# northflank-examples/distributed-pytorch-example

Hardware: AMD Instinct MI355X
Metric: samples/sec (whole node) + DDP scaling eff., ResNet-50 bf16 at 1/2/4/8 MI355X (higher is better)
Workload: dtype bf16; 1 GPU; model=resnet50-v1.5, global_batch=512, per_gpu_batch=512, grad_accum=1, parallelism=dp1, optimizer=sgd-momentum0.9

## Files before the change

### csrc/bindings/bn.cpp

```cpp
#include <algorithm>
#include <vector>

#include "../kernels/pwconv.h"
#include "gemm_plan.h"
#include "ops_common.h"

namespace dpe_ops {
namespace {

int64_t rows_of(const Tensor& x) { return x.numel() / x.size(-1); }

std::vector<Tensor> bn_fwd_train(const Tensor& x, const c10::optional<Tensor>& gamma, const c10::optional<Tensor>& beta,
                                 const c10::optional<Tensor>& rmean, const c10::optional<Tensor>& rvar, double momentum,
                                 double eps, bool relu, const c10::optional<Tensor>& residual,
                                 const c10::optional<Tensor>& stats) {
  CHECK_GPU(x); CHECK_BF16(x); CHECK_CONTIG(x);
  const int64_t C = x.size(-1), M = rows_of(x);
  TORCH_CHECK(C % 8 == 0 && C <= 2048, "bn: C must be a multiple of 8 and <= 2048");
  auto fo = x.options().dtype(at::kFloat);
  Tensor coef = at::empty({4, C}, fo);
  hipStream_t st = cur_stream();
  if (has(stats)) {
    TORCH_CHECK(stats->dim() == 3 && stats->size(0) == 2 && stats->size(1) == C, "stats must be [2][C][nb] partials");
    CHECK_RC(dpe_bn_finalize(fp(*stats), (int)stats->size(2), (int)C, M, fpo(gamma), fpo(beta), fpom(rmean), fpom(rvar),
                             (float)momentum, (float)eps, fp(coef), st), "bn_finalize");
  } else {
    const int nb = dpe_bn_stats_nblocks(M, (int)C);
    Tensor part = at::empty({nb, 2, C}, fo);
    CHECK_RC(dpe_bn_stats(bp(x), M, (int)C, nb, fp(part), st), "bn_stats");
    CHECK_RC(dpe_bn_finalize(fp(part), nb, (int)C, M, fpo(gamma), fpo(beta), fpom(rmean), fpom(rvar), (float)momentum,
                             (float)eps, fp(coef), st), "bn_finalize");
  }
  Tensor y = at::empty_like(x);
  const uint16_t* res = nullptr;
  if (has(residual)) { CHECK_BF16((*residual)); CHECK_CONTIG((*residual)); res = bp(*residual); }
  CHECK_RC(dpe_bn_apply(bp(x), res, bpm(y), M, (int)C, fp(coef), relu ? 1 : 0, st), "bn_apply");
  return {y, coef};
}

Tensor bn_fwd_eval(const Tensor& x, const c10::optional<Tensor>& gamma, const c10::optional<Tensor>& beta,
                   const Tensor& rmean, const Tensor& rvar, double eps, bool relu, const c10::optional<Tensor>& residual) {
  CHECK_GPU(x); CHECK_BF16(x); CHECK_CONTIG(x);
  const int64_t C = x.size(-1), M = rows_of(x);
  Tensor coef = at::empty({4, C}, x.options().dtype(at::kFloat));
  hipStream_t st = cur_stream();
  CHECK_RC(dpe_bn_eval_coeff((int)C, fpo(gamma), fpo(beta), fp(rmean), fp(rvar), (float)eps, fp(coef), st), "bn_eval");
  Tensor y = at::empty_like(x);
  const uint16_t* res = nullptr;
  if (has(residual)) res = bp(*residual);
  CHECK_RC(dpe_bn_apply(bp(x), res, bpm(y), M, (int)C, fp(coef), relu ? 1 : 0, st), "bn_apply");
  return y;
}

std::vector<Tensor> bn_bwd(const Tensor& dy, const c10::optional<Tensor>& y, const Tensor& x,
                           const c10::optional<Tensor>& gamma, const Tensor& coef, const c10::optional<Tensor>& dgamma,
                           const c10::optional<Tensor>& dbeta, bool want_dz, const c10::optional<Tensor>& y_bits) {
  CHECK_GPU(dy); CHECK_BF16(dy); CHECK_CONTIG(dy); CHECK_CONTIG(x);
  const int64_t C = x.size(-1), M = rows_of(x);
  const uint16_t* yp = has(y) ? bp(*y) : nullptr;
  const uint8_t* yb = nullptr;
  if (has(y_bits)) {
    CHECK_CONTIG((*y_bits));
    TORCH_CHECK(y_bits->scalar_type() == at::kByte && y_bits->numel() * 8 == x.numel() && C % 8 == 0,
                "bn_bwd: y_bits must be uint8 mask bits [.., C/8] of x's shape");
    yb = (const uint8_t*)y_bits->data_ptr();
    yp = nullptr;
  }
  hipStream_t st = cur_stream();
  auto fo = x.options().dtype(at::kFloat);
  const int nb = dpe_bn_bwd_nblocks(M, (int)C);
  Tensor part = at::empty({nb, 2, C}, fo);
  CHECK_RC(dpe_bn_bwd_reduce(bp(dy), yp, yb, bp(x), fp(coef), M, (int)C, nb, fp(part), st), "bn_bwd_reduce");
  Tensor bcoef = at::empty({3, C}, fo);
  CHECK_RC(dpe_bn_bwd_finalize(fp(part), nb, (int)C, M, fpo(gamma), fp(coef), fpom(dgamma), fpom(dbeta), fp(bcoef), st),
           "bn_bwd_finalize");
  Tensor dx = at::empty_like(x);
  Tensor dz;
  if (want_dz) dz = at::empty_like(x);
  CHECK_RC(dpe_bn_bwd_apply(bp(dy), yp, yb, bp(x), fp(bcoef), bpm(dx), want_dz ? bpm(dz) : nullptr, M, (int)C, nullptr, st),
           "bn_bwd_apply");
  return {dx, dz};
}

std::vector<Tensor> bn_gram(const Tensor& x, const c10::optional<Tensor>& coef, const c10::optional<Tensor>& shift_coef,
                            bool stride2) {
  CHECK_GPU(x); CHECK_BF16(x); CHECK_CONTIG(x);
  TORCH_CHECK(!stride2 || (x.dim() == 4 && x.size(1) % 2 == 0 && x.size(2) % 2 == 0), "bn_gram: stride2 needs [N, H, W, C], even H, W");
  const int64_t C = x.size(-1), M = x.numel() / C / (stride2 ? 4 : 1);
  TORCH_CHECK(C == 64 || C == 128 || C == 256, "bn_gram: C must be 64, 128 or 256");
  if (has(coef)) {
    CHECK_F32((*coef)); CHECK_CONTIG((*coef));
    TORCH_CHECK(coef->numel() >= 2 * C, "bn_gram: coef must be the BN's [4][C] coefficients");
  }
  const float* scoef = fpo(coef);
  if (scoef) TORCH_CHECK(coef->numel() == 4 * C, "bn_gram: the shift needs coef's full [4][C] (scale, shift, mean, invstd)");
  if (has(shift_coef)) {
    CHECK_F32((*shift_coef)); CHECK_CONTIG((*shift_coef));
    TORCH_CHECK(shift_coef->numel() == 4 * C, "bn_gram: shift_coef must be the BN's [4][C] coefficients");
    scoef = fp(*shift_coef);
  }
  auto fo = x.options().dtype(at::kFloat);
  Tensor ws = at::empty({dpe_gram_ws_floats(M, (int)C)}, fo);
  Tensor G = at::empty({C, C}, fo), sv = at::empty({2, C}, fo);
  CHECK_RC(dpe_gram(bp(x), fpo(coef), scoef, M, (int)C, fp(ws), fp(G), fp(sv), cur_stream(), stride2 ? (int)x.size(1) : 0,
                    stride2 ? (int)x.size(2) : 0), "bn_gram");
  return {G, sv};
}

std::vector<Tensor> bn_gram_coef(const Tensor& G, const Tensor& sv, const Tensor& w, int64_t M,
                                 const c10::optional<Tensor>& gamma, const c10::optional<Tensor>& beta,
                                 const c10::optional<Tensor>& rmean, const c10::optional<Tensor>& rvar, double momentum,
                                 double eps) {
  CHECK_GPU(G); CHECK_F32(G); CHECK_F32(sv); CHECK_BF16(w); CHECK_CONTIG(w); CHECK_CONTIG(G);
  const int64_t Cin = G.size(0), Cout = w.size(0);
  TORCH_CHECK(w.numel() == Cout * Cin && sv.numel() == 2 * Cin, "bn_gram_coef: shapes (s is bn_gram's [2][C])");
  CHECK_CONTIG(sv);
  Tensor coef = at::empty({4, Cout}, G.options()), u = at::empty({Cout, Cin}, G.options());
  CHECK_RC(dpe_gram_coef(fp(G), fp(sv), bp(w), (int)Cin, (int)Cout, M, fpo(gamma), fpo(beta), fpom(rmean), fpom(rvar),
                         (float)momentum, (float)eps, fp(coef), fp(u), cur_stream()), "bn_gram_coef");
  return {coef, u};
}

std::vector<Tensor> conv1x1_apply(const Tensor& x, const Tensor& w, const c10::optional<Tensor>& in_coef,
                                  const Tensor& out_coef, const Tensor& residual, const c10::optional<Tensor>& res_coef) {
  CHECK_GPU(x); CHECK_BF16(x); CHECK_CONTIG(x); CHECK_BF16(w); CHECK_CONTIG(w); CHECK_F32(out_coef);
  CHECK_BF16(residual); CHECK_CONTIG(residual);
  const int64_t K = x.size(-1), M = x.numel() / K, N = w.size(0);
  TORCH_CHECK(w.numel() == N * K && out_coef.numel() == 4 * N, "conv1x1_apply: shapes");
  auto ysz = x.sizes().vec();
  ysz.back() = N;
  TORCH_CHECK(residual.sizes().vec() == ysz, "conv1x1_apply: residual must have the output's shape");
  const int rg = pw_stream_on() ? dpe_pw_rowgroups(M, N, K, dpe::PW_APPLY) : 0;
  TORCH_CHECK(rg > 0, "conv1x1_apply: outside the streaming pointwise kernel's envelope");
  Tensor y = at::empty(ysz, x.options());
  auto bsz = ysz;
  bsz.back() = N / 8;
  Tensor bits = at::empty(bsz, x.options().dtype(at::kByte));
  dpe::PwArgs pa{};
  pa.x = bp(x); pa.w = bp(w); pa.y = bpm(y);
  pa.in_coef = fpo(in_coef);
  pa.out_coef = fp(out_coef);
  pa.residual = bp(residual);
  pa.res_coef = fpo(res_coef);
  pa.out_bits = (uint8_t*)bits.data_ptr();
  pa.M = M; pa.N = N; pa.K = K; pa.rg = rg; pa.sched = dpe_gemm::sched_buffer(cur_stream());
  CHECK_RC(dpe_pw_launch(&pa, dpe::PW_APPLY, cur_stream()), "pw_stream apply");
  return {y, bits};
}

std::vector<Tensor> bn_gram_bwd(const Tensor& part, const Tensor& P, const Tensor& w, const Tensor& u, const Tensor& sv,
                                const Tensor& coef, const c10::optional<Tensor>& gamma, int64_t M,
                                const c10::optional<Tensor>& dgamma, const c10::optional<Tensor>& dbeta, Tensor& dw) {
  CHECK_GPU(part); CHECK_F32(part); CHECK_F32(P); CHECK_F32(u); CHECK_F32(sv); CHECK_F32(coef); CHECK_F32(dw);
  CHECK_BF16(w); CHECK_CONTIG(w); CHECK_CONTIG(P); CHECK_CONTIG(dw); CHECK_CONTIG(part);
  const int64_t Cout = w.size(0), Cin = w.numel() / Cout;
  TORCH_CHECK(part.dim() == 3 && part.size(1) == Cout && P.numel() == Cout * Cin && u.numel() == Cout * Cin &&
                  dw.numel() == Cout * Cin && sv.numel() == 2 * Cin && coef.numel() == 4 * Cout && sv.is_contiguous(),
              "bn_gram_bwd: shapes");
  auto fo = P.options();
  Tensor bcat = at::empty({Cout + Cin, Cin}, w.options()), abc = at::empty({3, Cout}, fo), e = at::empty({Cin}, fo);
  Tensor qws = at::empty({dpe_gram_bwd_ws_floats((int)Cin, (int)Cout)}, fo);
  CHECK_RC(dpe_gram_bwd(fp(part), (int)part.size(2), fp(P), bp(w), fp(u), fp(sv), fp(coef), fpo(gamma), (int)Cin,
                        (int)Cout, M, fpom(dgamma), fpom(dbeta), fp(dw), bpm(bcat), fp(abc), fp(e), fp(qws), cur_stream()),
           "bn_gram_bwd");
  return {bcat, e};
}

std::vector<Tensor> conv1x1_dgrad_cat(const Tensor& dz, const Tensor& a2src, const c10::optional<Tensor>& a2_coef,
                                      const Tensor& bcat, const Tensor& e, const Tensor& bn_x, const Tensor& bn_coef) {
  CHECK_GPU(dz); CHECK_BF16(dz); CHECK_CONTIG(dz); CHECK_BF16(a2src); CHECK_CONTIG(a2src); CHECK_BF16(bcat);
  CHECK_CONTIG(bcat); CHECK_F32(e); CHECK_BF16(bn_x); CHECK_CONTIG(bn_x); CHECK_F32(bn_coef);
  const int64_t K1 = dz.size(-1), M = dz.numel() / K1, C = a2src.size(-1);
  TORCH_CHECK(a2src.numel() == M * C && bcat.size(0) == K1 + C && bcat.size(1) == C && e.numel() == C &&
                  bn_x.sizes() == a2src.sizes() && bn_coef.numel() == 4 * C && K1 % 32 == 0 && C % 32 == 0,
              "conv1x1_dgrad_cat: shapes");
  Tensor dx = at::empty_like(bn_x);
  if (hgemm_conv_on() && !has(a2_coef) && C >= 256 && C % 64 == 0 && K1 % 64 == 0) {
    int pcols = 0;
    const auto pl = dpe_gemm::plan_bnb(M, C, K1 + C, 1, 0, &pcols);
    if (pl.cfg >= 0 && pl.splits == 1 && pcols > 0) {
      Tensor part = at::empty({2, C, pcols}, dz.options().dtype(at::kFloat));
      auto h = hargs();
      h.A = bp(dz); h.B = bp(bcat); h.C = dx.data_ptr();
      h.M = (int)M; h.N = (int)C; h.K = (int)(K1 + C);
      h.lda = K1; h.ldb = C; h.ldc = C;
      h.bias = fp(e);
      h.conv = 3; h.A2 = bp(a2src); h.lda2 = C; h.k1 = (int)K1;
      h.col_stats = fp(part); h.stats_ld = pcols; h.st_x = bp(bn_x); h.st_coef = fp(bn_coef);
      dpe_gemm::run_bnb(h, pl, 1, 0);
      return {dx, part};
    }
  }
  if (has(a2_coef) && a2src.data_ptr() == bn_x.data_ptr() && a2_coef->numel() == 4 * C &&
      bn_coef.data_ptr() == a2_coef->data_ptr()) {
    const int rg = dpe_pw_cat_blocks(M, K1, C);
    if (rg > 0) {
      Tensor part = at::empty({2, C, rg}, dz.options().dtype(at::kFloat));
      dpe::PwCatArgs pa{};
      pa.dz = bp(dz); pa.h2 = bp(a2src); pa.coef = fp(bn_coef); pa.bcat = bp(bcat); pa.ebias = fp(e);
      pa.y = bpm(dx); pa.stats = fp(part); pa.M = M; pa.rg = rg;
      CHECK_RC(dpe_pw_cat_launch(&pa, K1, C, cur_stream()), "pw_cat data grad");
      return {dx, part};
    }
  }
  auto a = base_args();
  a.A = bp(dz); a.B = bp(bcat); a.C = dx.data_ptr();
  a.M = (int)M; a.N = (int)C; a.K = (int)(K1 + C);
  a.lda = K1; a.ldb = C; a.ldc = C;
  a.k_split = a.K;
  a.bias = fp(e);
  a.a_mode = dpe::AX_CAT;
  a.a2 = bp(a2src); a.lda2 = C; a.k1 = (int)K1;
  a.a_coef = fpo(a2_coef);
  a.st_x = bp(bn_x); a.st_coef = fp(bn_coef);
  const int bm = 128, bn = C <= 64 ? 64 : 128;
  const int64_t tilesM = (M + bm - 1) / bm;
  Tensor part = at::empty({2, C, tilesM}, dz.options().dtype(at::kFloat));
  a.col_stats = fp(part);
  a.stats_ld = (int)tilesM;
  const int rc = dpe_igemm_dma_launch(&a, bm, bn, dpe::A_DENSE_K, dpe::B_DENSE_N, dpe::EPI_BF16_BNB, cur_stream());
  CHECK_RC(rc, "igemm_dma AX_CAT data grad");
  return {dx, part};
}

Tensor bn_gram_pilot(const Tensor& x, bool stride2) {
  CHECK_GPU(x); CHECK_BF16(x); CHECK_CONTIG(x);
  TORCH_CHECK(!stride2 || (x.dim() == 4 && x.size(1) % 2 == 0 && x.size(2) % 2 == 0), "bn_gram_pilot: stride2 needs [N, H, W, C], even H, W");
  const int64_t C = x.size(-1), M = x.numel() / C / (stride2 ? 4 : 1);
  TORCH_CHECK(C == 64 || C == 128 || C == 256, "bn_gram_pilot: C must be 64, 128 or 256");
  Tensor coef = at::empty({4, C}, x.options().dtype(at::kFloat));
  CHECK_RC(dpe_gram_pilot(bp(x), M, (int)C, fp(coef), cur_stream(), stride2 ? (int)x.size(1) : 0,
                          stride2 ? (int)x.size(2) : 0), "bn_gram_pilot");
  return coef;
}

Tensor bn_gram_u(const Tensor& G, const Tensor& w) {
  CHECK_GPU(G); CHECK_F32(G); CHECK_CONTIG(G); CHECK_BF16(w); CHECK_CONTIG(w);
  const int64_t Cin = G.size(0), Cout = w.size(0);
  TORCH_CHECK(G.dim() == 2 && G.size(1) == Cin && w.numel() == Cout * Cin, "bn_gram_u: shapes");
  Tensor u = at::empty({Cout, Cin}, G.options());
  CHECK_RC(dpe_gram_u(fp(G), bp(w), (int)Cin, (int)Cout, fp(u), cur_stream()), "bn_gram_u");
  return u;
}

Tensor conv1x1_dgrad_cat_plain(const Tensor& dz, const Tensor& x, const Tensor& bcat, const Tensor& e, bool stride2) {
  CHECK_GPU(dz); CHECK_BF16(dz); CHECK_CONTIG(dz); CHECK_BF16(x); CHECK_CONTIG(x); CHECK_BF16(bcat); CHECK_CONTIG(bcat);
  CHECK_F32(e);
  const int64_t K1 = dz.size(-1), M = dz.numel() / K1, C = x.size(-1);
  if (stride2) {
    TORCH_CHECK(x.dim() == 4 && dz.dim() == 4 && x.size(1) == 2 * dz.size(1) && x.size(2) == 2 * dz.size(2) &&
                    x.size(0) == dz.size(0) && bcat.dim() == 2 && bcat.size(0) == K1 + C && bcat.size(1) == C &&
                    e.numel() == C && K1 % 32 == 0 && C % 32 == 0,
                "conv1x1_dgrad_cat_plain: stride-2 shapes");
    Tensor dx = at::empty({dz.size(0), dz.size(1), dz.size(2), C}, x.options());
    auto a = base_args();
    a.A = bp(dz); a.B = bp(bcat); a.C = dx.data_ptr();
    a.M = (int)M; a.N = (int)C; a.K = (int)(K1 + C);
    a.lda = K1; a.ldb = C; a.ldc = C;
    a.k_split = a.K;
    a.bias = fp(e);
    a.a_mode = dpe::AX_CAT;
    a.a2 = bp(x); a.lda2 = C; a.k1 = (int)K1;
    a.a2_h = (int)x.size(1); a.a2_w = (int)x.size(2);
    CHECK_RC(dpe_igemm_dma_launch(&a, 128, C <= 64 ? 64 : 128, dpe::A_DENSE_K, dpe::B_DENSE_N, dpe::EPI_BF16, cur_stream()),
             "igemm_dma AX_CAT data grad (stride-2 second segment)");
    return dx;
  }
  TORCH_CHECK(x.numel() == M * C && bcat.dim() == 2 && bcat.size(0) == K1 + C && bcat.size(1) == C && e.numel() == C,
              "conv1x1_dgrad_cat_plain: shapes");
  const int rg = dpe_pw_cat_blocks(M, K1, C);
  TORCH_CHECK(rg > 0, "conv1x1_dgrad_cat_plain: outside the streaming concatenated-K kernel's envelope");
  Tensor dx = at::empty_like(x);
  dpe::PwCatArgs pa{};
  pa.dz = bp(dz); pa.h2 = bp(x); pa.bcat = bp(bcat); pa.ebias = fp(e);
  pa.y = bpm(dx); pa.M = M; pa.rg = rg;
  CHECK_RC(dpe_pw_cat_launch(&pa, K1, C, cur_stream()), "pw_cat data grad (plain)");
  return dx;
}

Tensor bn_coef(const Tensor& stats, int64_t M, const c10::optional<Tensor>& gamma, const c10::optional<Tensor>& beta,
               const c10::optional<Tensor>& rmean, const c10::optional<Tensor>& rvar, double momentum, double eps) {
  CHECK_GPU(stats); CHECK_F32(stats);
  TORCH_CHECK(stats.dim() == 3 && stats.size(0) == 2, "stats must be [2][C][nb] partials");
  const int64_t C = stats.size(1);
  Tensor coef = at::empty({4, C}, stats.options());
  CHECK_RC(dpe_bn_finalize(fp(stats), (int)stats.size(2), (int)C, M, fpo(gamma), fpo(beta), fpom(rmean), fpom(rvar),
                           (float)momentum, (float)eps, fp(coef), cur_stream()), "bn_finalize");
  return coef;
}

Tensor bn_bwd_partials(const Tensor& dy, const Tensor& x, const c10::optional<Tensor>& gamma, const Tensor& coef,
                       const Tensor& partials, const c10::optional<Tensor>& dgamma, const c10::optional<Tensor>& dbeta,
                       bool relu_mask) {
  CHECK_GPU(dy); CHECK_BF16(dy); CHECK_CONTIG(dy); CHECK_CONTIG(x); CHECK_BF16(x);
  TORCH_CHECK(dy.sizes() == x.sizes(), "bn_bwd_partials: dy/x shape mismatch");
  const int64_t C = x.size(-1), M = rows_of(x);
  TORCH_CHECK(partials.dim() == 3 && partials.size(0) == 2 && partials.size(1) == C, "partials must be [2][C][nb]");
  hipStream_t st = cur_stream();
  Tensor bcoef = at::empty({3, C}, x.options().dtype(at::kFloat));
  CHECK_RC(dpe_bn_bwd_finalize(fp(partials), (int)partials.size(2), (int)C, M, fpo(gamma), fp(coef), fpom(dgamma),
                               fpom(dbeta), fp(bcoef), st), "bn_bwd_finalize");
  Tensor dx = at::empty_like(x);
  CHECK_RC(dpe_bn_bwd_apply(bp(dy), nullptr, nullptr, bp(x), fp(bcoef), bpm(dx), nullptr, M, (int)C, relu_mask ? fp(coef) : nullptr, st),
           "bn_bwd_apply");
  return dx;
}

Tensor bn_bwd_coef(const Tensor& partials, int64_t M, const c10::optional<Tensor>& gamma, const Tensor& coef,
                   const c10::optional<Tensor>& dgamma, const c10::optional<Tensor>& dbeta) {
  CHECK_GPU(partials); CHECK_F32(partials);
  TORCH_CHECK(partials.dim() == 3 && partials.size(0) == 2, "partials must be [2][C][nb]");
  const int64_t C = partials.size(1);
  Tensor bcoef = at::empty({3, C}, partials.options());
  CHECK_RC(dpe_bn_bwd_finalize(fp(partials), (int)partials.size(2), (int)C, M, fpo(gamma), fp(coef), fpom(dgamma),
                               fpom(dbeta), fp(bcoef), cur_stream()), "bn_bwd_finalize");
  return bcoef;
}

std::vector<Tensor> conv1x1_bnin_fwd(const Tensor& h, const Tensor& res, const Tensor& coef,
                                     const c10::optional<Tensor>& res_coef, const Tensor& w, Tensor& x_out,
                                     Tensor& x_bits, bool want_stats, int64_t tile_m) {
  CHECK_GPU(h); CHECK_BF16(h); CHECK_BF16(res); CHECK_BF16(w); CHECK_BF16(x_out);
  CHECK_CONTIG(h); CHECK_CONTIG(res); CHECK_CONTIG(w); CHECK_CONTIG(x_out); CHECK_CONTIG(x_bits);
  CHECK_F32(coef);
  TORCH_CHECK(h.dim() == 4 && w.dim() == 4 && w.size(1) == 1 && w.size(2) == 1 && w.size(3) == h.size(3),
              "conv1x1_bnin_fwd: NHWC h / [K,1,1,C] w shape mismatch");
  TORCH_CHECK(res.sizes() == h.sizes() && x_out.sizes() == h.sizes(), "conv1x1_bnin_fwd: res / x_out must have h's shape");
  TORCH_CHECK(x_bits.scalar_type() == at::kByte && x_bits.numel() * 8 == h.numel(), "conv1x1_bnin_fwd: x_bits [.., C/8] u8");
  const int64_t C = h.size(3), K = w.size(0);
  TORCH_CHECK(coef.numel() == 4 * C && (!res_coef.has_value() || res_coef->numel() == 4 * C), "coef must be [4][C]");
  TORCH_CHECK(C % 32 == 0 && C <= 2048 && K % 8 == 0, "conv1x1_bnin_fwd: C % 32 == 0, C <= 2048");
  Tensor y = at::empty({h.size(0), h.size(1), h.size(2), K}, h.options());
  auto a = base_args();
  a.g = geom(h, w, 1, 1, 0, 0, 1, 1, h.size(1), h.size(2));
  a.A = bp(h); a.B = bp(w); a.C = y.data_ptr();
  a.M = (int)(h.numel() / C); a.N = (int)K; a.K = (int)C;
  a.lda = C; a.ldb = C; a.ldc = K;
  a.k_split = a.K;
  a.a_mode = has(res_coef) ? dpe::AX_BN_RES2 : dpe::AX_BN_RES;
  a.a2 = bp(res); a.a_coef = fp(coef); a.a_coef2 = fpo(res_coef);
  a.a_out = bpm(x_out); a.a_bits = (uint8_t*)x_bits.data_ptr();
  Tensor stats;
  if (want_stats) {
    stats = at::empty({2, K, (a.M + 127) / 128}, h.options().dtype(at::kFloat));
    a.col_stats = fp(stats);
  }
  const int bm = (K == 64 && tile_m == 256) ? 256 : 128, bn = K <= 64 ? 64 : 128;
  CHECK_RC(dpe_igemm_dma_launch(&a, bm, bn, dpe::A_DENSE_K, dpe::B_DENSE_K, dpe::EPI_BF16, cur_stream()),
           "conv1x1_bnin_fwd");
  return {y, stats};
}

std::vector<Tensor> conv1x1_bnin_dgrad(const Tensor& dz, const Tensor& h, const Tensor& bcoef, const Tensor& w,
                                       Tensor& dh_out, const Tensor& bn_x, const Tensor& bn_coef) {
  CHECK_GPU(dz); CHECK_BF16(dz); CHECK_BF16(h); CHECK_BF16(w); CHECK_BF16(dh_out); CHECK_BF16(bn_x);
  CHECK_CONTIG(dz); CHECK_CONTIG(h); CHECK_CONTIG(w); CHECK_CONTIG(dh_out); CHECK_CONTIG(bn_x);
  CHECK_F32(bcoef); CHECK_F32(bn_coef);
  TORCH_CHECK(dz.dim() == 4 && w.dim() == 4 && w.size(1) == 1 && w.size(2) == 1 && w.size(0) == dz.size(3),
              "conv1x1_bnin_dgrad: NHWC dz / [K,1,1,C] w shape mismatch");
  TORCH_CHECK(h.sizes() == dz.sizes() && dh_out.sizes() == dz.sizes(), "conv1x1_bnin_dgrad: h / dh_out must have dz's shape");
  const int64_t K = dz.size(3), C = w.size(3);
  TORCH_CHECK(bcoef.numel() == 3 * K, "bcoef must be [3][K]");
  TORCH_CHECK(K % 32 == 0 && K <= 2048 && C % 8 == 0, "conv1x1_bnin_dgrad: K % 32 == 0, K <= 2048");
  TORCH_CHECK(bn_x.dim() == 4 && bn_x.size(0) == dz.size(0) && bn_x.size(1) == dz.size(1) && bn_x.size(2) == dz.size(2) &&
                  bn_x.size(3) == C && bn_coef.numel() == 4 * C,
              "conv1x1_bnin_dgrad: bn_x must be [N,H,W,C], bn_coef [4][C]");
  Tensor dx = at::empty_like(bn_x);
  auto a = base_args();
  a.g = geom(dx, w, 1, 1, 0, 0, 1, 1, dz.size(1), dz.size(2));
  a.A = bp(dz); a.B = bp(w); a.C = dx.data_ptr();
  a.M = (int)(dz.numel() / K); a.N = (int)C; a.K = (int)K;
  a.lda = K; a.ldb = C; a.ldc = C;
  a.k_split = a.K;
  a.a_mode = dpe::AX_BN_BWD;
  a.a2 = bp(h); a.a_coef = fp(bcoef); a.a_out = bpm(dh_out);
  a.st_x = bp(bn_x); a.st_coef = fp(bn_coef);
  const int64_t tiles_m = (a.M + 127) / 128;
  Tensor part = at::empty({2, C, tiles_m}, dz.options().dtype(at::kFloat));
  a.col_stats = fp(part);
  a.stats_ld = (int)tiles_m;
  const int bn = C <= 64 ? 64 : 128;
  CHECK_RC(dpe_igemm_dma_launch(&a, 128, bn, dpe::A_DENSE_K, dpe::B_DENSE_N, dpe::EPI_BF16_BNB, cur_stream()),
           "conv1x1_bnin_dgrad");
  return {dx, part};
}

std::vector<Tensor> bn_bwd_dual(const Tensor& dz, const Tensor& x, const c10::optional<Tensor>& gamma, const Tensor& coef,
                                const Tensor& partials, const c10::optional<Tensor>& dgamma,
                                const c10::optional<Tensor>& dbeta, const Tensor& x2, const c10::optional<Tensor>& gamma2,
                                const Tensor& coef2, const c10::optional<Tensor>& dgamma2, const c10::optional<Tensor>& dbeta2) {
  CHECK_GPU(dz); CHECK_BF16(dz); CHECK_CONTIG(dz); CHECK_BF16(x); CHECK_CONTIG(x); CHECK_BF16(x2); CHECK_CONTIG(x2);
  TORCH_CHECK(dz.sizes() == x.sizes() && dz.sizes() == x2.sizes(), "bn_bwd_dual: dz / x / x2 shape mismatch");
  const int64_t C = x.size(-1), M = rows_of(x);
  TORCH_CHECK(partials.dim() == 3 && partials.size(0) == 2 && partials.size(1) == C, "partials must be [2][C][nb]");
  hipStream_t st = cur_stream();
  auto fo = x.options().dtype(at::kFloat);
  Tensor bcoef = at::empty({3, C}, fo);
  CHECK_RC(dpe_bn_bwd_finalize(fp(partials), (int)partials.size(2), (int)C, M, fpo(gamma), fp(coef), fpom(dgamma),
                               fpom(dbeta), fp(bcoef), st), "bn_bwd_finalize");
  const int nb = dpe_bn_bwd_nblocks(M, (int)C);
  Tensor part2 = at::empty({2, C, nb}, fo);
  Tensor dx = at::empty_like(x);
  CHECK_RC(dpe_bn_bwd_reduce_apply(bp(dz), bp(x2), fp(coef2), bp(x), fp(bcoef), bpm(dx), M, (int)C, nb, fp(part2), st),
           "bn_bwd_reduce_apply");
  Tensor bcoef2 = at::empty({3, C}, fo);
  CHECK_RC(dpe_bn_bwd_finalize(fp(part2), nb, (int)C, M, fpo(gamma2), fp(coef2), fpom(dgamma2), fpom(dbeta2), fp(bcoef2), st),
           "bn_bwd_finalize");
  Tensor dx2 = at::empty_like(x2);
  CHECK_RC(dpe_bn_bwd_apply(bp(dz), nullptr, nullptr, bp(x2), fp(bcoef2), bpm(dx2), nullptr, M, (int)C, nullptr, st),
           "bn_bwd_apply");
  return {dx, dx2};
}

std::vector<Tensor> maxpool_fwd(const Tensor& x, int64_t k, int64_t s, int64_t p) {
  CHECK_GPU(x); CHECK_BF16(x); CHECK_CONTIG(x);
  const int64_t N = x.size(0), H = x.size(1), W = x.size(2), C = x.size(3);
  const int64_t OH = (H + 2 * p - k) / s + 1, OW = (W + 2 * p - k) / s + 1;
  Tensor y = at::empty({N, OH, OW, C}, x.options());
  Tensor idx = at::empty({N, OH, OW, C}, x.options().dtype(at::kByte));
  CHECK_RC(dpe_maxpool_fwd(bp(x), bpm(y), (uint8_t*)idx.data_ptr(), (int)N, (int)H, (int)W, (int)C, (int)OH, (int)OW, (int)k,
                           (int)s, (int)p, cur_stream()), "maxpool_fwd");
  return {y, idx};
}

Tensor maxpool_bwd(const Tensor& dy, const Tensor& idx, std::vector<int64_t> xshape, int64_t k, int64_t s, int64_t p) {
  CHECK_GPU(dy); CHECK_BF16(dy); CHECK_CONTIG(dy);
  Tensor dx = at::empty(xshape, dy.options());
  CHECK_RC(dpe_maxpool_bwd(bp(dy), (const uint8_t*)idx.data_ptr(), bpm(dx), (int)xshape[0], (int)xshape[1], (int)xshape[2],
                           (int)xshape[3], (int)dy.size(1), (int)dy.size(2), (int)k, (int)s, (int)p, cur_stream()),
           "maxpool_bwd");
  return dx;
}

std::vector<Tensor> bn_apply(const Tensor& x, const Tensor& coef, const c10::optional<Tensor>& residual,
                             const c10::optional<Tensor>& residual_coef, bool relu, bool want_mask) {
  CHECK_GPU(x); CHECK_BF16(x); CHECK_CONTIG(x); CHECK_F32(coef);
  const int64_t C = x.size(-1);
  TORCH_CHECK(C % 8 == 0 && coef.numel() == 4 * C, "bn_apply: coef must be [4][C], C % 8 == 0");
  const bool has_res = has(residual);
  if (has_res) {
    CHECK_BF16((*residual)); CHECK_CONTIG((*residual));
    TORCH_CHECK(residual->sizes() == x.sizes(), "bn_apply: residual shape mismatch");
  }
  Tensor y = at::empty_like(x);
  Tensor bits;
  if (want_mask) {
    auto sz = x.sizes().vec();
    sz.back() = C / 8;
    bits = at::empty(sz, x.options().dtype(at::kByte));
  }
  uint8_t* mb = want_mask ? (uint8_t*)bits.data_ptr() : nullptr;
  if (has(residual_coef)) {
    TORCH_CHECK(has_res, "bn_apply: residual_coef needs a residual");
    CHECK_F32((*residual_coef));
    TORCH_CHECK(residual_coef->numel() == 4 * C, "bn_apply: residual_coef must be [4][C]");
    CHECK_RC(dpe_bn_apply2(bp(x), fp(coef), bp(*residual), fp(*residual_coef), bpm(y), rows_of(x), (int)C, relu ? 1 : 0, mb,
                           cur_stream()), "bn_apply2");
  } else {
    CHECK_RC(dpe_bn_apply_m(bp(x), has_res ? bp(*residual) : nullptr, bpm(y), rows_of(x), (int)C, fp(coef), relu ? 1 : 0, mb,
                            cur_stream()), "bn_apply");
  }
  return {y, bits};
}

std::vector<Tensor> bnrelu_maxpool_fwd(const Tensor& h, const Tensor& coef, int64_t k, int64_t s, int64_t p) {
  CHECK_GPU(h); CHECK_BF16(h); CHECK_CONTIG(h); CHECK_F32(coef);
  const int64_t N = h.size(0), H = h.size(1), W = h.size(2), C = h.size(3);
  TORCH_CHECK(coef.numel() == 4 * C, "bnrelu_maxpool_fwd: coef must be [4][C]");
  const int64_t OH = (H + 2 * p - k) / s + 1, OW = (W + 2 * p - k) / s + 1;
  Tensor y = at::empty({N, OH, OW, C}, h.options());
  Tensor idx = at::empty({N, OH, OW, C}, h.options().dtype(at::kByte));
  CHECK_RC(dpe_bnrelu_maxpool_fwd(bp(h), fp(coef), bpm(y), (uint8_t*)idx.data_ptr(), (int)N, (int)H, (int)W, (int)C, (int)OH,
                                  (int)OW, (int)k, (int)s, (int)p, cur_stream()), "bnrelu_maxpool_fwd");
  return {y, idx};
}

Tensor maxpool_bn_bwd(const Tensor& dy, const Tensor& idx, const Tensor& h, const c10::optional<Tensor>& gamma,
                      const Tensor& coef, const c10::optional<Tensor>& dgamma, const c10::optional<Tensor>& dbeta, int64_t k,
                      int64_t s, int64_t p) {
  CHECK_GPU(dy); CHECK_BF16(dy); CHECK_CONTIG(dy); CHECK_BF16(h); CHECK_CONTIG(h); CHECK_F32(coef);
  TORCH_CHECK(idx.scalar_type() == at::kByte && idx.sizes() == dy.sizes(), "maxpool_bn_bwd: idx must be uint8 of dy's shape");
  const int64_t N = h.size(0), H = h.size(1), W = h.size(2), C = h.size(3);
  TORCH_CHECK(dy.size(0) == N && dy.size(3) == C, "maxpool_bn_bwd: dy/h shape mismatch");
  const int64_t M = N * H * W;
  hipStream_t st = cur_stream();
  auto fo = h.options().dtype(at::kFloat);
  const int nb = (int)std::max<int64_t>(1, std::min<int64_t>(8192, M / 512));
  Tensor part = at::empty({2, C, nb}, fo);
  CHECK_RC(dpe_maxpool_bn_bwd_reduce(bp(dy), (const uint8_t*)idx.data_ptr(), bp(h), fp(coef), (int)N, (int)H, (int)W, (int)C,
                                     (int)dy.size(1), (int)dy.size(2), (int)k, (int)s, (int)p, nb, fp(part), st),
           "maxpool_bn_bwd_reduce");
  Tensor bcoef = at::empty({3, C}, fo);
  CHECK_RC(dpe_bn_bwd_finalize(fp(part), nb, (int)C, M, fpo(gamma), fp(coef), fpom(dgamma), fpom(dbeta), fp(bcoef), st),
           "bn_bwd_finalize");
  Tensor dh = at::empty_like(h);
  CHECK_RC(dpe_maxpool_bn_bwd_apply(bp(dy), (const uint8_t*)idx.data_ptr(), bp(h), fp(coef), fp(bcoef), bpm(dh), (int)N,
                                    (int)H, (int)W, (int)C, (int)dy.size(1), (int)dy.size(2), (int)k, (int)s, (int)p, st),
           "maxpool_bn_bwd_apply");
  return dh;
}

void stem_bwd_fused(const Tensor& dy, const Tensor& idx, const Tensor& h, const Tensor& xs,
                    const c10::optional<Tensor>& gamma, const Tensor& coef, const c10::optional<Tensor>& dgamma,
                    const c10::optional<Tensor>& dbeta, Tensor& dw) {
  CHECK_GPU(dy); CHECK_BF16(dy); CHECK_CONTIG(dy); CHECK_BF16(h); CHECK_CONTIG(h); CHECK_F32(coef); CHECK_BF16(xs);
  CHECK_CONTIG(xs); CHECK_F32(dw); CHECK_CONTIG(dw);
  TORCH_CHECK(idx.scalar_type() == at::kByte && idx.sizes() == dy.sizes(), "stem_bwd_fused: idx must be uint8 of dy's shape");
  const int64_t N = h.size(0), H = h.size(1), W = h.size(2), C = h.size(3);
  TORCH_CHECK(C == 64 && dy.size(0) == N && dy.size(1) == H / 2 && dy.size(2) == W / 2 && dy.size(3) == C && H % 2 == 0 &&
                  W % 2 == 0 && xs.size(0) == N && xs.size(1) == H && xs.size(2) == W && xs.size(3) == 16 &&
                  dw.numel() == 64 * 256,
              "stem_bwd_fused: shapes (h [N,H,W,64], dy/idx [N,H/2,W/2,64], xs [N,H,W,16], dw [64,4,4,16])");
  const int64_t M = N * H * W;
  hipStream_t st = cur_stream();
  auto fo = h.options().dtype(at::kFloat);
  const int nb = (int)std::max<int64_t>(1, std::min<int64_t>(8192, M / 512));
  Tensor part = at::empty({2, C, nb}, fo);
  CHECK_RC(dpe_maxpool_bn_bwd_reduce(bp(dy), (const uint8_t*)idx.data_ptr(), bp(h), fp(coef), (int)N, (int)H, (int)W, (int)C,
                                     (int)dy.size(1), (int)dy.size(2), 3, 2, 1, nb, fp(part), st),
           "maxpool_bn_bwd_reduce");
  Tensor bcoef = at::empty({3, C}, fo);
  CHECK_RC(dpe_bn_bwd_finalize(fp(part), nb, (int)C, M, fpo(gamma), fp(coef), fpom(dgamma), fpom(dbeta), fp(bcoef), st),
           "bn_bwd_finalize");
  auto scratch = at::empty({dpe_stem_wgrad_scratch(N, H, W)}, fo);
  CHECK_RC(dpe_stem_wgrad_launch2(bp(xs), nullptr, fp(dw), fp(scratch), (int)N, (int)H, (int)W, 1.f, bp(dy),
                                  (const uint8_t*)idx.data_ptr(), bp(h), fp(coef), fp(bcoef), st),
           "stem wgrad (fused BN / max-pool backward)");
}

Tensor gavgpool_fwd(const Tensor& x) {
  CHECK_GPU(x); CHECK_BF16(x); CHECK_CONTIG(x);
  const int64_t N = x.size(0), C = x.size(-1), HW = x.numel() / (N * C);
  Tensor y = at::empty({N, C}, x.options());
  CHECK_RC(dpe_gavgpool_fwd(bp(x), bpm(y), (int)N, (int)HW, (int)C, cur_stream()), "gavgpool_fwd");
  return y;
}

Tensor gavgpool_bwd(const Tensor& dy, std::vector<int64_t> xshape) {
  CHECK_GPU(dy); CHECK_BF16(dy); CHECK_CONTIG(dy);
  Tensor dx = at::empty(xshape, dy.options());
  const int64_t N = xshape[0], C = xshape.back(), HW = dx.numel() / (N * C);
  CHECK_RC(dpe_gavgpool_bwd(bp(dy), bpm(dx), (int)N, (int)HW, (int)C, cur_stream()), "gavgpool_bwd");
  return dx;
}

}

void register_bn(pybind11::module& m) {
  namespace py = pybind11;
  m.def("gram_ok", [](std::vector<int64_t> h2shape, int64_t cout3, int64_t next_width) {
          if (h2shape.size() != 4 || !pw_stream_on()) return false;
          const int64_t M = h2shape[0] * h2shape[1] * h2shape[2], C2 = h2shape[3];
          if (C2 != 64 && C2 != 128 && C2 != 256) return false;
          if (cout3 % 128 || M % 32) return false;
          return dpe_pw_rowgroups(M, cout3, C2, dpe::PW_APPLY) > 0 &&
                 dpe_pw_rowgroups(M, cout3, next_width, dpe::PW_DSUM) > 0;
        }, py::arg("h2_shape"), py::arg("cout3"), py::arg("next_width"));
  m.def("bn_gram", &bn_gram, py::arg("x"), py::arg("coef") = py::none(), py::arg("shift_coef") = py::none(),
        py::arg("stride2") = false,
        "(G = a'^T a', s = [colsum(a'), mu]) of a' = a2 - mu, a2 = relu(x * coef[0] + coef[1]) (or x), centred on the "
        "pilot shift of shift_coef (default coef); fp32, deterministic");
  m.def("bn_gram_coef", &bn_gram_coef, py::arg("G"), py::arg("s"), py::arg("w"), py::arg("M"), py::arg("gamma"),
        py::arg("beta"), py::arg("running_mean"), py::arg("running_var"), py::arg("momentum"), py::arg("eps"),
        "BN coefficients [4][Cout] of the never-computed h = a2 W^T from (G, s), and u = W G");
  m.def("conv1x1_apply", &conv1x1_apply, py::arg("x"), py::arg("w"), py::arg("in_coef"), py::arg("out_coef"),
        py::arg("residual"), py::arg("res_coef") = py::none(),
        "y = relu(BN(x' W^T) + residual [BN_d]) and its ReLU bits (pre-BN tensor never stored)");
  m.def("bn_gram_bwd", &bn_gram_bwd, py::arg("part"), py::arg("P"), py::arg("w"), py::arg("u"), py::arg("s"),
        py::arg("coef"), py::arg("gamma"), py::arg("M"), py::arg("dgamma"), py::arg("dbeta"), py::arg("dw"),
        "BN3 backward from (sum dz partials, P = dz^T a2): dgamma/dbeta/dw +=, returns (B_cat bf16, bias)");
  m.def("conv1x1_dgrad_cat", &conv1x1_dgrad_cat, py::arg("dz"), py::arg("a2src"), py::arg("a2_coef"), py::arg("bcat"),
        py::arg("e"), py::arg("bn_x"), py::arg("bn_coef"),
        "[dz | a2] x bcat + e with the BN2-backward partials (concatenated-K data grad)");
  m.def("bn_gram_pilot", &bn_gram_pilot, py::arg("x"), py::arg("stride2") = false,
        "pilot shift [4][C] for bn_gram's shift_coef from a sample of x's rows (x without a producing BN)");
  m.def("bn_gram_u", &bn_gram_u, py::arg("G"), py::arg("w"), "u = W G (fp32) alone: no coefficients, no running stats");
  m.def("conv1x1_dgrad_cat_plain", &conv1x1_dgrad_cat_plain, py::arg("dz"), py::arg("x"), py::arg("bcat"), py::arg("e"),
        py::arg("stride2") = false,
        "[dz | x] x bcat + e (concatenated-K data grad of a Gram-path downsample branch, no partials)");
  m.def("bnd_gram_ok", [](std::vector<int64_t> xshape, int64_t cout, std::vector<int64_t> stride) {
          if (xshape.size() != 4 || stride.size() != 2 || stride[0] != stride[1] || !igemm_dma_on()) return false;
          const int64_t M = xshape[0] * xshape[1] * xshape[2], C = xshape[3];
          if (stride[0] == 1) return (C == 64 || C == 128) && cout == 4 * C && dpe_pw_cat_blocks(M, cout, C) > 0;
          if (stride[0] != 2 || xshape[1] % 2 || xshape[2] % 2) return false;
          static const bool gdma = env_on("DPE_GRAM_DMA", true);
          const int64_t Mo = M / 4, lim = (1ll << 31) - 4096;
          return gdma && (C == 64 || C == 128 || C == 256) && cout >= 256 && cout % 32 == 0 && hgemm_conv_on() &&
                 hgemm_conv_wgrad_on() && Mo % 64 == 0 && Mo < (1 << 24) && M * C * 2 < lim && Mo * cout * 2 < lim;
        }, py::arg("xshape"), py::arg("cout"), py::arg("stride"));
  m.def("bn_bwd_coef", &bn_bwd_coef, py::arg("partials"), py::arg("M"), py::arg("gamma"), py::arg("coef"),
        py::arg("dgamma") = py::none(), py::arg("dbeta") = py::none(),
        "BN-backward coefficients [3][C] from the dgrad-epilogue partials (no apply pass); dgamma/dbeta +=");
  m.def("conv1x1_bnin_fwd", &conv1x1_bnin_fwd, py::arg("h"), py::arg("res"), py::arg("coef"), py::arg("res_coef"),
        py::arg("w"), py::arg("x_out"), py::arg("x_bits"), py::arg("want_stats") = true, py::arg("tile_m") = 128,
        "1x1 conv over x = relu(BN(h) + res [BN_d]) computed on load; x (+ ReLU bits) stored as a by-product");
  m.def("conv1x1_bnin_dgrad", &conv1x1_bnin_dgrad, py::arg("dz"), py::arg("h"), py::arg("bcoef"), py::arg("w"),
        py::arg("dh_out"), py::arg("bn_x"), py::arg("bn_coef"),
        "1x1 data grad over dh = a*dz + b*h + c computed on load (dh stored as a by-product) + BN-backward partials");
  m.def("bn_coef", &bn_coef, py::arg("stats"), py::arg("M"), py::arg("gamma"), py::arg("beta"), py::arg("running_mean"),
        py::arg("running_var"), py::arg("momentum"), py::arg("eps"));
  m.def("bn_apply", &bn_apply, py::arg("x"), py::arg("coef"), py::arg("residual") = py::none(),
        py::arg("residual_coef") = py::none(), py::arg("relu") = true, py::arg("want_mask") = false);
  m.def("bnrelu_maxpool_fwd", &bnrelu_maxpool_fwd, py::arg("h"), py::arg("coef"), py::arg("k"), py::arg("s"), py::arg("p"));
  m.def("set_pool_legacy", [](bool on) { dpe_set_pool_legacy(on ? 1 : 0); },
        "test hook: the stem max-pool on the reference (per-tap compare) kernel instead of the key-max one");
  m.def("stem_bwd_fused", &stem_bwd_fused, py::arg("dy"), py::arg("idx"), py::arg("h"), py::arg("xs"), py::arg("gamma"),
        py::arg("coef"), py::arg("dgamma"), py::arg("dbeta"), py::arg("dw"),
        "stem backward without dY: BN-backward coefficients of the pooled gradient, then the stem weight grad "
        "(s2d filter layout) computing dY on the fly");
  m.def("maxpool_bn_bwd", &maxpool_bn_bwd, py::arg("dy"), py::arg("idx"), py::arg("h"), py::arg("gamma"), py::arg("coef"),
        py::arg("dgamma"), py::arg("dbeta"), py::arg("k"), py::arg("s"), py::arg("p"));
  m.def("bn_bwd_partials", &bn_bwd_partials, py::arg("dy"), py::arg("x"), py::arg("gamma"), py::arg("coef"),
        py::arg("partials"), py::arg("dgamma") = py::none(), py::arg("dbeta") = py::none(), py::arg("relu_mask") = true);
  m.def("bn_fwd_train", &bn_fwd_train, py::arg("x"), py::arg("gamma"), py::arg("beta"), py::arg("rmean"), py::arg("rvar"),
        py::arg("momentum"), py::arg("eps"), py::arg("relu"), py::arg("residual") = py::none(), py::arg("stats") = py::none());
  m.def("bn_fwd_eval", &bn_fwd_eval, py::arg("x"), py::arg("gamma"), py::arg("beta"), py::arg("rmean"), py::arg("rvar"),
        py::arg("eps"), py::arg("relu"), py::arg("residual") = py::none());
  m.def("bn_bwd_dual", &bn_bwd_dual, py::arg("dz"), py::arg("x"), py::arg("gamma"), py::arg("coef"), py::arg("partials"),
        py::arg("dgamma"), py::arg("dbeta"), py::arg("x2"), py::arg("gamma2"), py::arg("coef2"), py::arg("dgamma2"),
        py::arg("dbeta2"), "backward of two BatchNorms fed by one dz (BN3 + downsample BN): dz read once for both");
  m.def("bn_bwd", &bn_bwd, py::arg("dy"), py::arg("y"), py::arg("x"), py::arg("gamma"), py::arg("coef"), py::arg("dgamma"),
        py::arg("dbeta"), py::arg("want_dz") = false, py::arg("y_bits") = py::none());
  m.def("maxpool_fwd", &maxpool_fwd);
  m.def("maxpool_bwd", &maxpool_bwd);
  m.def("gavgpool_fwd", &gavgpool_fwd);
  m.def("gavgpool_bwd", &gavgpool_bwd);
}

}
```

### csrc/kernels/pwconv.h

```cpp
#pragma once
#include <hip/hip_runtime.h>
#include <stdint.h>

namespace dpe {

enum PwEpi : int {
  PW_FWD = 0,
  PW_DGRAD = 1,
  PW_APPLY = 2,
  PW_DSUM = 3,
};

struct PwArgs {
  const uint16_t* x;
  const uint16_t* w;
  uint16_t* y;
  float* stats;
  const uint16_t* residual;
  const uint8_t* res_mask;
  const uint16_t* st_x;
  const float* st_coef;
  const uint8_t* st_mask;
  int64_t M, N, K;
  int rg;
  const float* in_coef;
  int res_h, res_w;
  const float* out_coef;
  const float* res_coef;
  uint8_t* out_bits;
  unsigned* sched;
  const uint16_t* p_src;
  const float* p_coef;
  float* p_slab;
  int p_k2;
};

struct PwCatArgs {
  const uint16_t* dz;
  const uint16_t* h2;
  const float* coef;
  const uint16_t* bcat;
  const float* ebias;
  uint16_t* y;
  float* stats;
  int64_t M;
  int rg;
};

}

extern "C" int dpe_pw_cat_blocks(int64_t M, int64_t K1, int64_t K2);
extern "C" int dpe_pw_cat_launch(const dpe::PwCatArgs* args, int64_t K1, int64_t K2, hipStream_t stream);

extern "C" int dpe_pw_rowgroups(int64_t M, int64_t N, int64_t K, int epi);
extern "C" int dpe_pw_launch(const dpe::PwArgs* args, int epi, hipStream_t stream);

extern "C" int dpe_pw_p_rowgroups(int64_t M, int64_t N, int64_t K, int64_t k2);
extern "C" int dpe_pw_p_reduce(const float* slab, int rg, int64_t n, float* P, hipStream_t stream);
```

### csrc/kernels/pwconv.hip

```cpp
#include <algorithm>
#include <cstdlib>

#include "common.h"
#include "igemm.h"
#include "launch.h"
#include "pwconv.h"

namespace dpe {
namespace pw {

constexpr int BM = 64;
typedef __attribute__((address_space(3))) void lds_void_t;

DPE_DEVICE int kimg_off(int row, int chunk) {
  const int g = (0x78 >> (((row >> 2) & 3) << 1)) & 3;
  return row * 64 + ((chunk ^ g) << 4);
}
DPE_DEVICE bf16x8 kfrag(const char* img, int r0) {
  const int lane = threadIdx.x & 63;
  return __builtin_bit_cast(bf16x8, *(const u32x4*)(img + kimg_off(r0 + (lane & 15), lane >> 4)));
}
DPE_DEVICE __amdgpu_buffer_rsrc_t rsrc(const void* base, uint32_t bytes) {
  return __builtin_amdgcn_make_buffer_rsrc(const_cast<void*>(base), (short)0, (int)bytes, 0x00020000);
}
template <int N>
DPE_DEVICE void wait_vm() {
  static_assert(N >= 0 && N < 64, "vmcnt");
  asm volatile("" ::: "memory");
  __builtin_amdgcn_s_waitcnt((N & 15) | (7 << 4) | (15 << 8) | ((N >> 4) << 14));
  asm volatile("" ::: "memory");
}

template <int C>
DPE_DEVICE int p_h(int row) {
  return C >= 128 ? ((row & 3) | (((row >> 3) & 1) << 2)) : (((row >> 1) & 1) | (((row >> 3) & 1) << 1));
}
typedef __attribute__((address_space(3))) s16x4 lds_s16x4_t;
DPE_DEVICE bf16x8 p_trfrag(const char* a1, const char* a2) {
  const s16x4 lo = __builtin_amdgcn_ds_read_tr16_b64_v4i16((lds_s16x4_t*)a1);
  const s16x4 hi = __builtin_amdgcn_ds_read_tr16_b64_v4i16((lds_s16x4_t*)a2);
  s16x8 r;
  r[0] = lo[0]; r[1] = lo[1]; r[2] = lo[2]; r[3] = lo[3];
  r[4] = hi[0]; r[5] = hi[1]; r[6] = hi[2]; r[7] = hi[3];
  return __builtin_bit_cast(bf16x8, r);
}

template <int K, int WN, int NS, int EPI, bool DYN = false, int K2 = 0>
__global__ __launch_bounds__(256, (K == 64 && (EPI == PW_FWD || (K2 > 0 && !DYN))) ? 3 : 2) void pw_stream_kernel(PwArgs a) {
  constexpr int KC = K / 32;
  constexpr int TILE = BM * K * 2;
  constexpr int P = TILE / 1024 / 4;
  constexpr int NI = WN / 16, MI = BM / 16;
  static_assert(P >= 1 && P * 4096 == TILE, "pieces");
  constexpr int ROWB = WN * 2 + 16, CPRW = WN / 8, RPP = 64 / CPRW, NPS = 32 / RPP;
  constexpr int STG = 32 * ROWB;
  constexpr int S = (EPI == PW_APPLY ? 4 : 2) * NPS;
  constexpr int VM = (NS - 1) * S + (NS - 2) * P;
  static_assert(VM < 64, "vmcnt range");
  constexpr bool PF = K2 > 0;
  static_assert(!PF || (EPI == PW_DSUM && WN == 32 && (K2 == 64 || K2 == 128) && K2 <= K), "fused P: envelope");
  constexpr int A2OFF = NS * TILE + 4 * STG + 2 * K * 4 + 16, A2RB = 2 * (PF ? K2 : 8);
  __shared__ __attribute__((aligned(16))) char smem[A2OFF + (PF ? BM * A2RB : 0)];
  float* const bnin = (float*)(smem + NS * TILE + 4 * STG);
  int* const claim_slot = (int*)(smem + NS * TILE + 4 * STG + 2 * K * 4);

  constexpr bool DG = EPI == PW_DGRAD || EPI == PW_DSUM;
  const int tid = threadIdx.x, lane = tid & 63, g = lane >> 4, li = lane & 15;
  const int wid = __builtin_amdgcn_readfirstlane(tid >> 6);
  const int M = (int)a.M, N = (int)a.N, RG = a.rg;
  const int nbN = N / (4 * WN);
  const int bid = xcd_remap(blockIdx.x, gridDim.x);
  const int nb = bid % nbN;
  int rg = bid / nbN;
  const int SRG = (int)gridDim.x / nbN;
  const int n0w = nb * 4 * WN + wid * WN;
  const int tiles = (M + BM - 1) / BM;
  const int ch = lane % CPRW;
  const int nch = n0w + ch * 8;

  bf16x8 wf[NI][KC];
#pragma unroll
  for (int ni = 0; ni < NI; ++ni)
#pragma unroll
    for (int kc = 0; kc < KC; ++kc) {
      const int n = n0w + 16 * ni + li, k0 = 32 * kc + 8 * g;
      if constexpr (!DG) {
        wf[ni][kc] = __builtin_bit_cast(bf16x8, *(const u32x4*)(a.w + (int64_t)n * K + k0));
      } else {
        s16x8 v;
#pragma unroll
        for (int e = 0; e < 8; ++e) v[e] = (short)a.w[(int64_t)(k0 + e) * N + n];
        wf[ni][kc] = __builtin_bit_cast(bf16x8, v);
      }
    }
  float bsc[8], bsh[8], bmu[8];
  const bool bnb = EPI == PW_DSUM || (EPI == PW_DGRAD && a.st_x != nullptr);
  const bool bnx = EPI == PW_DGRAD && a.st_x != nullptr;
  if (bnx) {
#pragma unroll
    for (int e = 0; e < 8; ++e) {
      bsc[e] = a.st_coef[nch + e];
      bsh[e] = a.st_coef[N + nch + e];
      bmu[e] = a.st_coef[2 * N + nch + e];
    }
  }

  const __amdgpu_buffer_rsrc_t xr = rsrc(a.x, (uint32_t)((int64_t)M * K * 2));
  uint32_t voff[P];
#pragma unroll
  for (int i = 0; i < P; ++i) {
    const int q = wid * P + i, kc = q >> 2, row = (q & 3) * 16 + (lane >> 2);
    const int lc = (lane & 3) ^ ((0x78 >> (((row >> 2) & 3) << 1)) & 3);
    voff[i] = (uint32_t)(row * K * 2 + kc * 64 + lc * 16);
  }
  auto issue = [&](int t, int slot) {
    char* dst = smem + slot * TILE;
    const int64_t base = t >= 0 ? (int64_t)t * BM * K * 2 : 0;
    const int valid_rows = t >= 0 ? M - t * BM : 0;
#pragma unroll
    for (int i = 0; i < P; ++i) {
      const int q = wid * P + i, row = (q & 3) * 16 + (lane >> 2);
      const uint32_t v = row < valid_rows ? voff[i] + (uint32_t)base : 0x80000000u;
      __builtin_amdgcn_raw_ptr_buffer_load_lds(xr, (lds_void_t*)(dst + q * 1024), 16, v, 0, 0, 0);
    }
  };

  float s[8], ss[8];
#pragma unroll
  for (int e = 0; e < 8; ++e) { s[e] = 0.f; ss[e] = 0.f; }
  constexpr int PNJ = PF ? K2 / 16 : 1, PCPR = PF ? K2 / 8 : 8, PRPP = 64 / PCPR, PPW = PCPR / 4;
  f32x4 pacc[NI][PNJ];
  if constexpr (PF) {
#pragma unroll
    for (int ni = 0; ni < NI; ++ni)
#pragma unroll
      for (int nj = 0; nj < PNJ; ++nj) pacc[ni][nj] = f32x4{0.f, 0.f, 0.f, 0.f};
  }
  float osc[8], osh[8], rsc[8], rsh[8];
  if constexpr (EPI == PW_APPLY) {
#pragma unroll
    for (int e = 0; e < 8; ++e) {
      osc[e] = a.out_coef[nch + e];
      osh[e] = a.out_coef[N + nch + e];
      rsc[e] = a.res_coef ? a.res_coef[nch + e] : 1.f;
      rsh[e] = a.res_coef ? a.res_coef[N + nch + e] : 0.f;
    }
  }
  const int rh = a.res_h, rw = a.res_w;
  auto res_off = [&](int m) -> int64_t {
    if (rh <= 0) return (int64_t)m * N + nch;
    const int hw = rh * rw, n = m / hw, r = m - n * hw, h = r / rw, w = r - h * rw;
    if ((h | w) & 1) return -1;
    return ((int64_t)(n * (rh >> 1) + (h >> 1)) * (rw >> 1) + (w >> 1)) * N + nch;
  };

  constexpr uint32_t OOB = 0xfffffff0u;
  const uint32_t ybytes = (uint32_t)((int64_t)M * N * 2), mbytes = (uint32_t)((int64_t)M * N / 8);
  const uint32_t rbytes = rh > 0 ? (uint32_t)((int64_t)(M / (rh * rw)) * (rh >> 1) * (rw >> 1) * N * 2) : ybytes;
  const __amdgpu_buffer_rsrc_t yrs = rsrc(a.y, ybytes);
  const __amdgpu_buffer_rsrc_t rrs = rsrc(a.residual, a.residual ? rbytes : 0u);
  const __amdgpu_buffer_rsrc_t rmrs = rsrc(a.res_mask, a.res_mask ? mbytes : 0u);
  const __amdgpu_buffer_rsrc_t xsrs = rsrc(a.st_x, bnx ? ybytes : 0u);
  const __amdgpu_buffer_rsrc_t smrs = rsrc(a.st_mask, (bnb && a.st_mask) ? mbytes : 0u);
  const __amdgpu_buffer_rsrc_t obrs = rsrc(a.out_bits, (EPI == PW_APPLY && a.out_bits) ? mbytes : 0u);
  const __amdgpu_buffer_rsrc_t psrs = rsrc(a.p_src, PF ? (uint32_t)((int64_t)M * K2 * 2) : 0u);

  if (!DG && a.in_coef) {
    for (int i = tid; i < 2 * K; i += 256) bnin[i] = a.in_coef[i];
    __syncthreads();
  }
  if constexpr (PF) {
    if (a.p_coef)
      for (int i = tid; i < 2 * K2; i += 256) bnin[i] = a.p_coef[i];
    __syncthreads();
  }

  auto tile_body = [&](const int m0, const int cur_slot, const int nxt_tile, const int nxt_slot) {
    constexpr bool HOIST = (EPI != PW_FWD) && (WN == 32);
    constexpr int HN = HOIST ? NPS : 1;
    u32x4 hrv[2][HN], hxv[2][HN];
    uint32_t hrmb[2][HN], hsmb[2][HN];
    if constexpr (HOIST) {
#pragma unroll
      for (int hf = 0; hf < 2; ++hf)
#pragma unroll
        for (int ps = 0; ps < HN; ++ps) {
          const int m = min(m0 + 32 * hf + ps * RPP + lane / CPRW, M - 1);
          const int64_t off = (int64_t)m * N + nch;
          const int64_t ro = EPI == PW_APPLY ? off : res_off(m);
          if (a.residual) hrv[hf][ps] = __builtin_amdgcn_raw_buffer_load_b128(rrs, ro >= 0 ? (uint32_t)(ro * 2) : OOB, 0, 0);
          if constexpr (DG) {
            if (a.res_mask) hrmb[hf][ps] = __builtin_amdgcn_raw_buffer_load_b8(rmrs, (uint32_t)(off >> 3), 0, 0);
            if (bnx) hxv[hf][ps] = __builtin_amdgcn_raw_buffer_load_b128(xsrs, (uint32_t)(off * 2), 0, 0);
            if (bnb && a.st_mask) hsmb[hf][ps] = __builtin_amdgcn_raw_buffer_load_b8(smrs, (uint32_t)(off >> 3), 0, 0);
          }
        }
    }
    if constexpr (PF) {
      int ol = lane;
      asm volatile("" : "+v"(ol));
#pragma unroll
      for (int k = 0; k < PPW; ++k) {
        const int q = wid * PPW + k, r = q * PRPP + ol / PCPR, lc = (ol % PCPR) ^ (2 * p_h<K2>(r));
        const int m = m0 + r;
        __builtin_amdgcn_raw_ptr_buffer_load_lds(psrs, (lds_void_t*)(smem + A2OFF + q * 1024), 16,
                                                 m < M ? (uint32_t)(((int64_t)m * K2 + 8 * lc) * 2) : 0x80000000u, 0, 0, 0);
      }
    }
    if (!DG && a.in_coef) {
      char* timg = smem + cur_slot * TILE;
#pragma unroll
      for (int q = 0; q < TILE / 16 / 256; ++q) {
        const int c = q * 256 + tid, kc = c / (BM * 4), rem = c % (BM * 4), row = rem >> 2, pc = rem & 3;
        const int lc = pc ^ ((0x78 >> (((row >> 2) & 3) << 1)) & 3);
        u32x4* pch = (u32x4*)(timg + kc * (BM * 64) + row * 64 + pc * 16);
        const f32x4* cs = (const f32x4*)(bnin + 32 * kc + 8 * lc);
        const f32x4* chh = (const f32x4*)(bnin + K + 32 * kc + 8 * lc);
        const f32x4 s0 = cs[0], s1 = cs[1], h0 = chh[0], h1 = chh[1];
        const float sc8[8] = {s0[0], s0[1], s0[2], s0[3], s1[0], s1[1], s1[2], s1[3]};
        const float sh8[8] = {h0[0], h0[1], h0[2], h0[3], h1[0], h1[1], h1[2], h1[3]};
        float f[8];
        unpack8(*pch, f);
#pragma unroll
        for (int e = 0; e < 8; ++e) f[e] = fmaxf(fmaf(f[e], sc8[e], sh8[e]), 0.f);
        *pch = pack8(f);
      }
      lds_barrier();
    }
    issue(nxt_tile, nxt_slot);
    const char* img = smem + cur_slot * TILE;
    f32x4 acc[MI][NI];
#pragma unroll
    for (int mi = 0; mi < MI; ++mi)
#pragma unroll
      for (int ni = 0; ni < NI; ++ni) acc[mi][ni] = f32x4{0.f, 0.f, 0.f, 0.f};
#pragma unroll
    for (int kc = 0; kc < KC; ++kc) {
      bf16x8 xf[MI];
#pragma unroll
      for (int mi = 0; mi < MI; ++mi) xf[mi] = kfrag(img + kc * (BM * 64), 16 * mi);
#pragma unroll
      for (int mi = 0; mi < MI; ++mi)
#pragma unroll
        for (int ni = 0; ni < NI; ++ni)
          acc[mi][ni] = __builtin_amdgcn_mfma_f32_16x16x32_bf16(wf[ni][kc], xf[mi], acc[mi][ni], 0, 0, 0);
    }
    if constexpr (PF) {
      wait_vm<P>();
      char* const a2 = smem + A2OFF;
      if (a.p_coef) {
        int ol = lane;
        asm volatile("" : "+v"(ol));
#pragma unroll
        for (int k = 0; k < PPW; ++k) {
          const int q = wid * PPW + k, r = q * PRPP + ol / PCPR, lc = (ol % PCPR) ^ (2 * p_h<K2>(r));
          const f32x4 s0 = *(const f32x4*)(bnin + 8 * lc), s1 = *(const f32x4*)(bnin + 8 * lc + 4);
          const f32x4 h0 = *(const f32x4*)(bnin + K2 + 8 * lc), h1 = *(const f32x4*)(bnin + K2 + 8 * lc + 4);
          const float sc8[8] = {s0[0], s0[1], s0[2], s0[3], s1[0], s1[1], s1[2], s1[3]};
          const float sh8[8] = {h0[0], h0[1], h0[2], h0[3], h1[0], h1[1], h1[2], h1[3]};
          u32x4* const pc = (u32x4*)(a2 + q * 1024 + ol * 16);
          float f[8];
          unpack8(*pc, f);
#pragma unroll
          for (int e = 0; e < 8; ++e) f[e] = fmaxf(fmaf(f[e], sc8[e], sh8[e]), 0.f);
          *pc = pack8(f);
        }
      }
    }
    char* stg = smem + NS * TILE + wid * STG;
#pragma unroll
    for (int hf = 0; hf < 2; ++hf) {
      u32x4 rv[NPS], xv[NPS];
      uint32_t rmb[NPS], smb[NPS];
      if constexpr (HOIST) {
#pragma unroll
        for (int ps = 0; ps < HN; ++ps) {
          rv[ps] = hrv[hf][ps];
          xv[ps] = hxv[hf][ps];
          rmb[ps] = a.res_mask ? hrmb[hf][ps] : 0xffu;
          smb[ps] = (bnb && a.st_mask) ? hsmb[hf][ps] : 0xffu;
        }
      } else if constexpr (DG) {
#pragma unroll
        for (int ps = 0; ps < NPS; ++ps) {
          const int m = min(m0 + 32 * hf + ps * RPP + lane / CPRW, M - 1);
          const int64_t off = (int64_t)m * N + nch;
          if (a.residual) {
            const int64_t ro = res_off(m);
            rv[ps] = ro >= 0 ? *(const u32x4*)(a.residual + ro) : u32x4{0u, 0u, 0u, 0u};
          }
          rmb[ps] = a.res_mask ? (uint32_t)a.res_mask[off >> 3] : 0xffu;
          if (bnx) xv[ps] = *(const u32x4*)(a.st_x + off);
          smb[ps] = (bnb && a.st_mask) ? (uint32_t)a.st_mask[off >> 3] : 0xffu;
        }
      }
#pragma unroll
      for (int mh = 0; mh < 2; ++mh) {
        const int mi = 2 * hf + mh;
#pragma unroll
        for (int ni = 0; ni < NI; ++ni) {
          u32x2 pk;
          pk[0] = pack_bf2(acc[mi][ni][0], acc[mi][ni][1]);
          pk[1] = pack_bf2(acc[mi][ni][2], acc[mi][ni][3]);
          *(u32x2*)(stg + (16 * mh + li) * ROWB + (16 * ni + 4 * g) * 2) = pk;
        }
      }
      if (HOIST && hf == 0) wait_vm<P>();
#pragma unroll
      for (int ps = 0; ps < NPS; ++ps) {
        const int row = ps * RPP + lane / CPRW;
        u32x4 v = *(const u32x4*)(stg + row * ROWB + ch * 16);
        const int m = m0 + 32 * hf + row;
        const bool valid = m < M;
        float f[8];
        unpack8(v, f);
        if constexpr (EPI == PW_APPLY) {
          float r[8];
          if (a.residual) unpack8(rv[ps], r);
#pragma unroll
          for (int e = 0; e < 8; ++e) {
            float t = fmaf(f[e], osc[e], osh[e]);
            if (a.residual) t += a.res_coef ? bf2f(f2bf(fmaf(r[e], rsc[e], rsh[e]))) : r[e];
            f[e] = fmaxf(t, 0.f);
          }
          v = pack8(f);
          if constexpr (HOIST)
            __builtin_amdgcn_raw_buffer_store_b8(relu_mask_byte(v), obrs, valid ? (uint32_t)(((int64_t)m * N + nch) >> 3) : OOB, 0, 0);
          else if (valid && a.out_bits)
            a.out_bits[((int64_t)m * N + nch) >> 3] = relu_mask_byte(v);
        } else if constexpr (EPI == PW_FWD) {
          const float vm = valid ? 1.f : 0.f;
#pragma unroll
          for (int e = 0; e < 8; ++e) {
            const float fv = f[e] * vm;
            s[e] += fv;
            ss[e] = fmaf(fv, fv, ss[e]);
          }
        } else {
          if (a.residual) {
            float r[8];
            unpack8(rv[ps], r);
#pragma unroll
            for (int e = 0; e < 8; ++e) f[e] += ((rmb[ps] >> e) & 1u) ? r[e] : 0.f;
            v = pack8(f);
            unpack8(v, f);
          }
          if (bnb && valid) {
            float x8[8];
            if (bnx) unpack8(xv[ps], x8);
            if (a.st_mask) {
#pragma unroll
              for (int e = 0; e < 8; ++e) {
                f[e] = ((smb[ps] >> e) & 1u) ? f[e] : 0.f;
                s[e] += f[e];
                if (bnx) ss[e] = fmaf(f[e], x8[e] - bmu[e], ss[e]);
              }
              v = pack8(f);
            } else {
#pragma unroll
              for (int e = 0; e < 8; ++e) {
                const float dz = fmaf(x8[e], bsc[e], bsh[e]) > 0.f ? f[e] : 0.f;
                s[e] += dz;
                ss[e] = fmaf(dz, x8[e] - bmu[e], ss[e]);
              }
            }
          }
        }
        if constexpr (HOIST) __builtin_amdgcn_raw_buffer_store_b128(v, yrs, valid ? (uint32_t)(((int64_t)m * N + nch) * 2) : OOB, 0, 0);
        else if (valid) *(u32x4*)(a.y + (int64_t)m * N + nch) = v;
        if constexpr (PF) *(u32x4*)(stg + row * ROWB + ch * 16) = valid ? v : u32x4{0u, 0u, 0u, 0u};
      }
      if constexpr (PF) {
        if (hf == 0) lds_barrier();
        else asm volatile("" ::: "memory");
        int ol = lane;
        asm volatile("" : "+v"(ol));
        const int g = ol >> 4, q4 = (ol >> 2) & 3, p4 = ol & 3;
        const char* const a2 = smem + A2OFF;
        bf16x8 ya[NI];
#pragma unroll
        for (int ni = 0; ni < NI; ++ni)
          ya[ni] = p_trfrag(stg + (8 * g + q4) * ROWB + (16 * ni + 4 * p4) * 2, stg + (8 * g + q4 + 4) * ROWB + (16 * ni + 4 * p4) * 2);
        const int r1 = 32 * hf + 8 * g + q4, r2 = r1 + 4;
        const int x1 = 2 * p_h<K2>(r1), x2 = 2 * p_h<K2>(r2);
#pragma unroll
        for (int nj = 0; nj < PNJ; ++nj) {
          const int c = 2 * nj + (p4 >> 1), sub = (p4 & 1) * 8;
          const bf16x8 bfr = p_trfrag(a2 + r1 * A2RB + ((c ^ x1) << 4) + sub, a2 + r2 * A2RB + ((c ^ x2) << 4) + sub);
#pragma unroll
          for (int ni = 0; ni < NI; ++ni)
            pacc[ni][nj] = __builtin_amdgcn_mfma_f32_16x16x32_bf16(ya[ni], bfr, pacc[ni][nj], 0, 0, 0);
        }
      }
    }
    if constexpr (PF) asm volatile("s_waitcnt lgkmcnt(0)" ::: "memory");
  };
  auto flush_stats = [&](int col) {
    if (EPI != PW_APPLY && a.stats) {
#pragma unroll
      for (int e = 0; e < 8; ++e) {
#pragma unroll
        for (int o = CPRW; o < 64; o <<= 1) {
          s[e] += __shfl_xor(s[e], o, 64);
          ss[e] += __shfl_xor(ss[e], o, 64);
        }
      }
      if (lane < CPRW) {
#pragma unroll
        for (int e = 0; e < 8; ++e) {
          a.stats[(int64_t)(nch + e) * RG + col] = s[e];
          if (EPI != PW_DSUM) a.stats[(int64_t)(N + nch + e) * RG + col] = ss[e];
        }
      }
#pragma unroll
      for (int e = 0; e < 8; ++e) { s[e] = 0.f; ss[e] = 0.f; }
    }
    if constexpr (PF) {
      float* const slab = a.p_slab + (int64_t)col * N * K2;
#pragma unroll
      for (int ni = 0; ni < NI; ++ni)
#pragma unroll
        for (int nj = 0; nj < PNJ; ++nj) {
#pragma unroll
          for (int e = 0; e < 4; ++e) slab[(int64_t)(n0w + 16 * ni + 4 * g + e) * K2 + 16 * nj + li] = pacc[ni][nj][e];
          pacc[ni][nj] = f32x4{0.f, 0.f, 0.f, 0.f};
        }
    }
  };
  auto ring_wait = [&](int p, bool ending) {
    if (ending) wait_vm<0>();
    else if (p == 0) wait_vm<(NS - 2) * P>();
    else if (NS >= 3 && p == 1) wait_vm<S + (NS - 2) * P>();
    else if (NS >= 4 && p == 2) wait_vm<2 * S + (NS - 2) * P>();
    else wait_vm<VM>();
    asm volatile("" ::: "memory");
    __builtin_amdgcn_s_barrier();
    asm volatile("" ::: "memory");
  };

  wait_vm<0>();
  if constexpr (!DYN) {
    const int nt = rg < tiles ? (tiles - 1 - rg) / RG + 1 : 0;
#pragma unroll
    for (int j = 0; j < NS - 1; ++j)
      if (j < nt) issue(rg + j * RG, j);
    for (int j = 0; j < nt; ++j) {
      ring_wait(j, j + NS - 2 >= nt);
      tile_body((rg + j * RG) * BM, j % NS, j + NS - 1 < nt ? rg + (j + NS - 1) * RG : -1, (j + NS - 1) % NS);
    }
    flush_stats(rg);
  } else {
    auto ntiles = [&](int u) { return (tiles - 1 - u) / RG + 1; };
    int cu = rg, ntc = ntiles(cu), jc = 0;
    int nu = -2;
    int iu = cu, ij = 0;
    int p = 0;
    int claimv = 0;
    auto next_issue = [&]() -> int {
      if (iu < 0) return -1;
      if (ij == ntiles(iu)) {
        iu = iu == cu ? nu : -1;
        ij = 0;
        if (iu < 0) return -1;
      }
      return iu + (ij++) * RG;
    };
    int issued = 0;
#pragma unroll
    for (int j = 0; j < NS - 1; ++j) {
      const int t = next_issue();
      if (t >= 0) { issue(t, j); ++issued; }
    }
    while (true) {
      ring_wait(p, issued < p + NS - 1);
      const int jpub = ntc - (NS + 1), jcl = max(0, jpub - 7);
      if (jc == jcl && tid == 0)
        claimv = SRG + (int)__hip_atomic_fetch_add(a.sched + nb * 256, 1u, __ATOMIC_RELAXED, __HIP_MEMORY_SCOPE_AGENT);
      if (jc == jpub && tid == 0) *claim_slot = claimv;
      if (jc == jpub + 1) {
        const int c = __builtin_amdgcn_readfirstlane(*claim_slot);
        nu = c < RG ? c : -1;
      }
      const int t = next_issue();
      if (t >= 0) ++issued;
      tile_body((cu + jc * RG) * BM, p % NS, t, (p + NS - 1) % NS);
      ++p;
      if (++jc == ntc) {
        flush_stats(cu);
        if (nu < 0) break;
        cu = nu;
        ntc = ntiles(cu);
        jc = 0;
        nu = -2;
      }
    }
    if (tid == 0) {
      if (__hip_atomic_fetch_add(a.sched + 16 * 256, 1u, __ATOMIC_RELAXED, __HIP_MEMORY_SCOPE_AGENT) == gridDim.x - 1u) {
        for (int k = 0; k < nbN; ++k) __hip_atomic_store(a.sched + k * 256, 0u, __ATOMIC_RELAXED, __HIP_MEMORY_SCOPE_AGENT);
        __hip_atomic_store(a.sched + 16 * 256, 0u, __ATOMIC_RELAXED, __HIP_MEMORY_SCOPE_AGENT);
      }
    }
  }
}

constexpr int CBM = 32;
template <int K1, int K2, int NS, bool BN = true>
__global__ __launch_bounds__(64 * (K2 / 16), K2 == 64 ? 2 : 1) void pw_cat_kernel(PwCatArgs a) {
  constexpr int NW = K2 / 16, NT = 64 * NW, N = K2;
  constexpr int KC1 = K1 / 32, KC2 = K2 / 32, KC = KC1 + KC2;
  constexpr int IMG = CBM * 64;
  constexpr int TILE = KC * IMG;
  constexpr int P = KC * 2 / NW;
  static_assert(P * NW == KC * 2, "piece split");
  constexpr int ROWB = 16 * 2 + 16;
  constexpr int STG = CBM * ROWB;
  constexpr int S = 1;
  constexpr int VM = (NS - 1) * S + (NS - 2) * P;
  static_assert(VM < 64, "vmcnt range");
  constexpr int A2B = BN ? KC2 * IMG : 0, BNB = BN ? 2 * K2 * 4 : 16;
  __shared__ __attribute__((aligned(16))) char smem[NS * TILE + A2B + NW * STG + BNB];
  float* const bnin = (float*)(smem + NS * TILE + A2B + NW * STG);
  char* const a2img = smem + NS * TILE;
  const int tid = threadIdx.x, lane = tid & 63, g = lane >> 4, li = lane & 15;
  const int wid = __builtin_amdgcn_readfirstlane(tid >> 6);
  const int M = (int)a.M, RG = a.rg;
  const int tiles = (M + CBM - 1) / CBM;
  const int n0w = wid * 16;
  char* const stg = smem + NS * TILE + A2B + wid * STG;
  auto swz = [](int row) { return (0x78 >> (((row >> 2) & 3) << 1)) & 3; };

  bf16x8 wf[KC];
#pragma unroll
  for (int kc = 0; kc < KC; ++kc) {
    s16x8 v;
#pragma unroll
    for (int e = 0; e < 8; ++e) v[e] = (short)a.bcat[(int64_t)(32 * kc + 8 * g + e) * N + n0w + li];
    wf[kc] = __builtin_bit_cast(bf16x8, v);
  }
  const int erow = lane >> 1, nch = n0w + 8 * (lane & 1);
  float eb[4], bsc[8], bsh[8], bmu[8];
#pragma unroll
  for (int e = 0; e < 4; ++e) eb[e] = a.ebias[n0w + 4 * g + e];
  if constexpr (BN) {
#pragma unroll
    for (int e = 0; e < 8; ++e) {
      bsc[e] = a.coef[nch + e];
      bsh[e] = a.coef[K2 + nch + e];
      bmu[e] = a.coef[2 * K2 + nch + e];
    }
    for (int i = tid; i < 2 * K2; i += NT) bnin[i] = a.coef[i];
  }

  const __amdgpu_buffer_rsrc_t r1 = rsrc(a.dz, (uint32_t)((int64_t)M * K1 * 2));
  const __amdgpu_buffer_rsrc_t r2 = rsrc(a.h2, (uint32_t)((int64_t)M * K2 * 2));
  uint32_t voff[P];
  int prow[P];
#pragma unroll
  for (int i = 0; i < P; ++i) {
    const int q = wid * P + i, kc = q >> 1, row = (q & 1) * 16 + (lane >> 2);
    const int lc = (lane & 3) ^ swz(row);
    prow[i] = row;
    voff[i] = kc < KC1 ? (uint32_t)(row * K1 * 2 + kc * 64 + lc * 16) : (uint32_t)(row * K2 * 2 + (kc - KC1) * 64 + lc * 16);
  }
  auto issue = [&](int t, int slot) {
    char* dst = smem + slot * TILE;
    const int valid_rows = M - t * CBM;
#pragma unroll
    for (int i = 0; i < P; ++i) {
      const int q = wid * P + i, kc = q >> 1;
      if (kc < KC1) {
        const uint32_t v = prow[i] < valid_rows ? voff[i] + (uint32_t)t * (CBM * K1 * 2) : 0x80000000u;
        __builtin_amdgcn_raw_ptr_buffer_load_lds(r1, (lds_void_t*)(dst + q * 1024), 16, v, 0, 0, 0);
      } else {
        const uint32_t v = prow[i] < valid_rows ? voff[i] + (uint32_t)t * (CBM * K2 * 2) : 0x80000000u;
        __builtin_amdgcn_raw_ptr_buffer_load_lds(r2, (lds_void_t*)(dst + q * 1024), 16, v, 0, 0, 0);
      }
    }
  };
  auto ring_wait = [&](int p, bool ending) {
    if (ending) wait_vm<0>();
    else if (p == 0) wait_vm<(NS - 2) * P>();
    else if (NS >= 3 && p == 1) wait_vm<S + (NS - 2) * P>();
    else wait_vm<VM>();
    asm volatile("" ::: "memory");
    __builtin_amdgcn_s_barrier();
    asm volatile("" ::: "memory");
  };

  float s[8], ss[8];
#pragma unroll
  for (int e = 0; e < 8; ++e) { s[e] = 0.f; ss[e] = 0.f; }
  const int rgb = blockIdx.x;
  const int nt = rgb < tiles ? (tiles - 1 - rgb) / RG + 1 : 0;
  wait_vm<0>();
  __syncthreads();
#pragma unroll
  for (int j = 0; j < NS - 1; ++j)
    if (j < nt) issue(rgb + j * RG, j);
  for (int j = 0; j < nt; ++j) {
    ring_wait(j, j + NS - 2 >= nt);
    const int slot = j % NS, m0 = (rgb + j * RG) * CBM;
    if (j + NS - 1 < nt) issue(rgb + (j + NS - 1) * RG, (j + NS - 1) % NS);
    const char* img = smem + slot * TILE;
    if constexpr (BN) {
#pragma unroll
    for (int c = tid; c < KC2 * CBM * 4; c += NT) {
      const int kc2 = c / (CBM * 4), rem = c % (CBM * 4), row = rem >> 2, pc = rem & 3;
      const int lc = pc ^ swz(row);
      const int off = kc2 * IMG + row * 64 + pc * 16;
      const f32x4* cs = (const f32x4*)(bnin + 32 * kc2 + 8 * lc);
      const f32x4* ch = (const f32x4*)(bnin + K2 + 32 * kc2 + 8 * lc);
      const f32x4 s0 = cs[0], s1 = cs[1], h0 = ch[0], h1 = ch[1];
      const float sc8[8] = {s0[0], s0[1], s0[2], s0[3], s1[0], s1[1], s1[2], s1[3]};
      const float sh8[8] = {h0[0], h0[1], h0[2], h0[3], h1[0], h1[1], h1[2], h1[3]};
      float f[8];
      unpack8(*(const u32x4*)(img + KC1 * IMG + off), f);
#pragma unroll
      for (int e = 0; e < 8; ++e) f[e] = fmaxf(fmaf(f[e], sc8[e], sh8[e]), 0.f);
      *(u32x4*)(a2img + off) = pack8(f);
    }
    lds_barrier();
    }
    f32x4 acc[2] = {f32x4{0.f, 0.f, 0.f, 0.f}, f32x4{0.f, 0.f, 0.f, 0.f}};
#pragma unroll
    for (int kc = 0; kc < KC; ++kc) {
      const char* im = (!BN || kc < KC1) ? img + kc * IMG : a2img + (kc - KC1) * IMG;
#pragma unroll
      for (int mi = 0; mi < 2; ++mi) acc[mi] = __builtin_amdgcn_mfma_f32_16x16x32_bf16(wf[kc], kfrag(im, 16 * mi), acc[mi], 0, 0, 0);
    }
#pragma unroll
    for (int mi = 0; mi < 2; ++mi) {
      u32x2 pk;
      pk[0] = pack_bf2(acc[mi][0] + eb[0], acc[mi][1] + eb[1]);
      pk[1] = pack_bf2(acc[mi][2] + eb[2], acc[mi][3] + eb[3]);
      *(u32x2*)(stg + (16 * mi + li) * ROWB + (4 * g) * 2) = pk;
    }
    const u32x4 v = *(const u32x4*)(stg + erow * ROWB + (lane & 1) * 16);
    const int m = m0 + erow;
    if (m < M) {
      if constexpr (BN) {
        float f[8], x8[8];
        unpack8(v, f);
        const int kc2 = nch >> 5, lc = (nch & 31) >> 3;
        unpack8(*(const u32x4*)(img + (KC1 + kc2) * IMG + erow * 64 + ((lc ^ swz(erow)) << 4)), x8);
#pragma unroll
        for (int e = 0; e < 8; ++e) {
          const float dz = fmaf(x8[e], bsc[e], bsh[e]) > 0.f ? f[e] : 0.f;
          s[e] += dz;
          ss[e] = fmaf(dz, x8[e] - bmu[e], ss[e]);
        }
      }
      *(u32x4*)(a.y + (int64_t)m * N + nch) = v;
    }
  }
  if constexpr (!BN) return;
#pragma unroll
  for (int e = 0; e < 8; ++e) {
#pragma unroll
    for (int o = 2; o < 64; o <<= 1) {
      s[e] += __shfl_xor(s[e], o, 64);
      ss[e] += __shfl_xor(ss[e], o, 64);
    }
  }
  if (lane < 2) {
#pragma unroll
    for (int e = 0; e < 8; ++e) {
      a.stats[(int64_t)(nch + e) * RG + rgb] = s[e];
      a.stats[(int64_t)(N + nch + e) * RG + rgb] = ss[e];
    }
  }
}

}
}

using namespace dpe;

extern "C" int dpe_pw_cat_blocks(int64_t M, int64_t K1, int64_t K2) {
  static const bool on = [] { const char* e = getenv("DPE_PW_CAT"); return !(e && e[0] == '0'); }();
  if (!on || !((K1 == 256 && K2 == 64) || (K1 == 512 && K2 == 128))) return 0;
  if (M <= 0 || M * K1 * 2 >= (1ll << 31) - 4096) return 0;
  int dev = 0, cus = 0;
  (void)hipGetDevice(&dev);
  (void)hipDeviceGetAttribute(&cus, hipDeviceAttributeMultiprocessorCount, dev);
  const int per = K2 == 64 ? 2 : 1;
  const int64_t tiles = (M + pw::CBM - 1) / pw::CBM;
  const int64_t nb = (int64_t)std::max(1, cus) * per * (dpe_cu_reserve() > 0 ? 2 : 1);
  return (int)std::max<int64_t>(1, std::min<int64_t>(nb, tiles));
}

extern "C" int dpe_pw_cat_launch(const PwCatArgs* args, int64_t K1, int64_t K2, hipStream_t st) {
  const PwCatArgs& a = *args;
  if (a.rg <= 0 || a.rg != dpe_pw_cat_blocks(a.M, K1, K2)) return -1;
  const bool bn = a.coef != nullptr;
  if (bn != (a.stats != nullptr)) return -1;
  if (K1 == 256 && K2 == 64) {
    if (bn) hipLaunchKernelGGL((pw::pw_cat_kernel<256, 64, 3>), dim3(a.rg), dim3(256), 0, st, a);
    else hipLaunchKernelGGL((pw::pw_cat_kernel<256, 64, 3, false>), dim3(a.rg), dim3(256), 0, st, a);
  } else if (K1 == 512 && K2 == 128) {
    if (bn) hipLaunchKernelGGL((pw::pw_cat_kernel<512, 128, 3>), dim3(a.rg), dim3(512), 0, st, a);
    else hipLaunchKernelGGL((pw::pw_cat_kernel<512, 128, 3, false>), dim3(a.rg), dim3(512), 0, st, a);
  } else {
    return -1;
  }
  return 0;
}

#ifndef DPE_PW64_DGRAD_WN
#define DPE_PW64_DGRAD_WN 32
#endif
#ifndef DPE_PW64_FWD_WN
#define DPE_PW64_FWD_WN 64
#endif
#ifndef DPE_PW128_FWD_WN
#define DPE_PW128_FWD_WN 64
#endif
static int pw_wn(int K, int epi) {
  if (epi == PW_APPLY) return 32;
  if (epi == PW_DSUM) epi = PW_DGRAD;
  if (K == 64) return epi == PW_DGRAD ? DPE_PW64_DGRAD_WN : DPE_PW64_FWD_WN;
  if (K == 128) return epi == PW_FWD ? DPE_PW128_FWD_WN : 32;
  return 32;
}

template <int K, int WN, int NS, int EPI, bool DYN, int K2 = 0>
static int pw_slots() {
  static int slots = [] {
    int dev = 0, cus = 0, per = 0;
    (void)hipGetDevice(&dev);
    (void)hipDeviceGetAttribute(&cus, hipDeviceAttributeMultiprocessorCount, dev);
    (void)hipOccupancyMaxActiveBlocksPerMultiprocessor(&per, pw::pw_stream_kernel<K, WN, NS, EPI, DYN, K2>, 256, 0);
    return std::max(1, per) * std::max(1, cus);
  }();
  return slots;
}
template <int EPI, bool DYN = false>
static int pw_capacity(int K) {
  if constexpr (EPI == PW_APPLY || EPI == PW_DSUM) {
    if (K == 64) return pw_slots<64, 32, 4, EPI, DYN>();
    if (K == 128) return pw_slots<128, 32, 3, EPI, DYN>();
    return pw_slots<256, 32, 2, EPI, DYN>();
  } else {
    if (K == 64) return EPI == PW_FWD ? pw_slots<64, DPE_PW64_FWD_WN, 4, EPI, DYN>() : pw_slots<64, DPE_PW64_DGRAD_WN, 4, EPI, DYN>();
    if (K == 128) return EPI == PW_FWD ? pw_slots<128, DPE_PW128_FWD_WN, 3, EPI, DYN>() : pw_slots<128, 32, 3, EPI, DYN>();
    return pw_slots<256, 32, 2, EPI, DYN>();
  }
}

static bool pw_dynamic() {
  static const bool on = [] { const char* e = getenv("DPE_PW_DYNAMIC"); return !(e && e[0] == '0'); }();
  return on;
}

static bool pw_p_shape(int64_t K, int64_t k2) { return (K == 64 && k2 == 64) || (K == 128 && (k2 == 64 || k2 == 128)); }
template <bool DYN>
static int pw_cap_p(int64_t K, int64_t k2) {
  if (K == 64 && k2 == 64) return pw_slots<64, 32, 4, PW_DSUM, DYN, 64>();
  if (K == 128 && k2 == 64) return pw_slots<128, 32, 3, PW_DSUM, DYN, 64>();
  if constexpr (!DYN)
    if (K == 128 && k2 == 128) return pw_slots<128, 32, 3, PW_DSUM, false, 128>();
  return 0;
}

template <bool DYN>
static int pw_cap(int64_t K, int epi, int64_t k2 = 0) {
  if (k2 > 0) return pw_cap_p<DYN>(K, k2);
  return epi == PW_FWD ? pw_capacity<PW_FWD, DYN>((int)K)
                       : epi == PW_APPLY ? pw_capacity<PW_APPLY, DYN>((int)K)
                       : epi == PW_DSUM  ? pw_capacity<PW_DSUM, DYN>((int)K) : pw_capacity<PW_DGRAD, DYN>((int)K);
}

struct PwPlan { int rg, srg; };
static PwPlan pw_plan(int64_t M, int64_t N, int64_t K, int epi, int64_t k2 = 0) {
  if (k2 > 0 && (epi != PW_DSUM || !pw_p_shape(K, k2))) return {0, 0};
  if (K != 64 && K != 128 && K != 256) return {0, 0};
  if (epi != PW_FWD && epi != PW_DGRAD && epi != PW_APPLY && epi != PW_DSUM) return {0, 0};
  const int bnb = 4 * pw_wn((int)K, epi);
  if (N % bnb || N < 2 * K) return {0, 0};
  if (M * K * 2 >= (1ll << 31) - 4096 || M * N >= (1ll << 31) - 256) return {0, 0};
  const int64_t tiles = (M + pw::BM - 1) / pw::BM;
  const int64_t nbN = N / bnb;
  const int reserve = dpe_cu_reserve();
  if (reserve > 0 && pw_dynamic()) {
    if (k2 == 128) return {0, 0};
    const int64_t srg = std::max<int64_t>(1, (pw_cap<true>(K, epi, k2) - reserve) / nbN);
    static const int64_t fac = [] { const char* e = getenv("DPE_PW_DYN_FACTOR"); return (int64_t)(e ? std::max(2, atoi(e)) : 8); }();
    const int64_t rg = std::min<int64_t>(fac * srg, tiles / 7);
    if (rg > srg) return {(int)rg, (int)srg};
  }
  int64_t rg = (pw_cap<false>(K, epi, k2) - reserve) / nbN;
  rg = std::max<int64_t>(1, std::min<int64_t>(rg, tiles));
  return {(int)rg, (int)rg};
}

extern "C" int dpe_pw_rowgroups(int64_t M, int64_t N, int64_t K, int epi) { return pw_plan(M, N, K, epi).rg; }

extern "C" int dpe_pw_p_rowgroups(int64_t M, int64_t N, int64_t K, int64_t k2) {
  return k2 > 0 ? pw_plan(M, N, K, PW_DSUM, k2).rg : 0;
}

__global__ __launch_bounds__(256) void pw_p_reduce_kernel(const float* __restrict__ slab, int rg, int64_t n,
                                                          float* __restrict__ P) {
  __shared__ float part[8][32];
  const int o = threadIdx.x & 31, q = threadIdx.x >> 5;
  const int64_t i = (int64_t)blockIdx.x * 32 + o;
  float t = 0.f;
  if (i < n) {
    int r = q;
    for (; r + 56 < rg; r += 64) {
      float v[8];
#pragma unroll
      for (int k = 0; k < 8; ++k) v[k] = slab[(int64_t)(r + 8 * k) * n + i];
#pragma unroll
      for (int k = 0; k < 8; ++k) t += v[k];
    }
    for (; r < rg; r += 8) t += slab[(int64_t)r * n + i];
  }
  part[q][o] = t;
  __syncthreads();
  if (q == 0 && i < n) {
    float u = 0.f;
#pragma unroll
    for (int k = 0; k < 8; ++k) u += part[k][o];
    P[i] = u;
  }
}

extern "C" int dpe_pw_p_reduce(const float* slab, int rg, int64_t n, float* P, hipStream_t st) {
  if (rg <= 0 || n <= 0) return -1;
  hipLaunchKernelGGL(pw_p_reduce_kernel, dim3((unsigned)((n + 31) / 32)), dim3(256), 0, st, slab, rg, n, P);
  return 0;
}

extern "C" int dpe_pw_launch(const PwArgs* args, int epi, hipStream_t st) {
  const PwArgs& a = *args;
  if (a.p_k2 < 0 || (a.p_k2 > 0 && (epi != PW_DSUM || !a.p_src || !a.p_slab))) return -1;
  if (a.rg <= 0 || a.rg != pw_plan(a.M, a.N, a.K, epi, a.p_k2).rg) return -1;
  if (epi == PW_FWD && (a.residual || a.st_x)) return -1;
  if (a.st_x && !a.st_coef) return -1;
  if (epi == PW_DSUM && (a.st_x || !a.st_mask || !a.stats)) return -1;
  if (epi == PW_APPLY && (!a.out_coef || a.st_x || a.stats || a.res_h > 0 || (a.res_coef && !a.residual))) return -1;
  if (a.res_h > 0 && ((epi != PW_DGRAD && epi != PW_DSUM) || a.res_mask || a.res_h % 2 || a.res_w % 2 || a.M % ((int64_t)a.res_h * a.res_w)))
    return -1;
  const int srg = a.sched ? pw_plan(a.M, a.N, a.K, epi, a.p_k2).srg : a.rg;
  const bool dyn = srg < a.rg;
  const int wn = pw_wn((int)a.K, epi);
  const dim3 grid((unsigned)(srg * (a.N / (4 * wn)))), block(256);
#define PW_GO(K_, WN_, NS_, E_)                                                                            \
  if (a.K == K_ && wn == WN_ && epi == E_) {                                                             \
    if (dyn) hipLaunchKernelGGL((pw::pw_stream_kernel<K_, WN_, NS_, E_, true>), grid, block, 0, st, a);    \
    else hipLaunchKernelGGL((pw::pw_stream_kernel<K_, WN_, NS_, E_, false>), grid, block, 0, st, a);       \
    return 0;                                                                                            \
  }
#define PW_GO_P(K_, NS_, K2_)                                                                                \
  if (a.K == K_ && a.p_k2 == K2_) {                                                                        \
    if (dyn) hipLaunchKernelGGL((pw::pw_stream_kernel<K_, 32, NS_, PW_DSUM, true, K2_>), grid, block, 0, st, a);  \
    else hipLaunchKernelGGL((pw::pw_stream_kernel<K_, 32, NS_, PW_DSUM, false, K2_>), grid, block, 0, st, a);     \
    return 0;                                                                                              \
  }
  if (a.p_k2 > 0) {
    PW_GO_P(64, 4, 64) PW_GO_P(128, 3, 64)
    if (a.K == 128 && a.p_k2 == 128 && !dyn) {
      hipLaunchKernelGGL((pw::pw_stream_kernel<128, 32, 3, PW_DSUM, false, 128>), grid, block, 0, st, a);
      return 0;
    }
    return -1;
  }
#undef PW_GO_P
  PW_GO(64, 32, 4, PW_APPLY) PW_GO(128, 32, 3, PW_APPLY) PW_GO(256, 32, 2, PW_APPLY)
  PW_GO(64, 32, 4, PW_DSUM) PW_GO(128, 32, 3, PW_DSUM) PW_GO(256, 32, 2, PW_DSUM)
  PW_GO(64, DPE_PW64_DGRAD_WN, 4, PW_DGRAD) PW_GO(64, DPE_PW64_FWD_WN, 4, PW_FWD)
  PW_GO(128, 32, 3, PW_DGRAD) PW_GO(128, DPE_PW128_FWD_WN, 3, PW_FWD)
  PW_GO(256, 32, 2, PW_DGRAD) PW_GO(256, 32, 2, PW_FWD)
#undef PW_GO
  return -1;
}
```

### distributed_pytorch_example_amd/models/_resnet_fused.py

```python
from __future__ import annotations

import os

import torch
from torch.autograd import Function

from ..ops._ext import ext
from ..ops._state import finalize_stream, grad_done, grad_sink, note_use, run_on_aux, shadow

_EPI_BNB = os.environ.get("DPE_BN_EPI", "1") != "0"
_BN3_CHAIN = _EPI_BNB and os.environ.get("DPE_BN3_CHAIN", "1") != "0"
_BN_DUAL = os.environ.get("DPE_BN_DUAL", "1") != "0"
_ROW_BNIN = _EPI_BNB and os.environ.get("DPE_ROW_BNIN", "1") != "0"
_PW_BNIN = _EPI_BNB and os.environ.get("DPE_PW_BNIN", "1") != "0"
_DOWN_CHAIN = _BN3_CHAIN and os.environ.get("DPE_DOWN_CHAIN", "1") != "0"
_AX_FWD = _BN3_CHAIN and os.environ.get("DPE_AX_FWD", "0") == "1"
_AX_BWD = _BN3_CHAIN and os.environ.get("DPE_AX_BWD", "0") == "1"
_AX_BWD_MAXC = int(os.environ.get("DPE_AX_BWD_MAXC", "512"))
_AX_TILE = int(os.environ.get("DPE_AX_TILE", "256"))
_GRAM = _BN3_CHAIN and os.environ.get("DPE_BN3_GRAM", "1") != "0"
_BND_GRAM = _GRAM and os.environ.get("DPE_BND_GRAM", "1") != "0"
_BND_GRAM_S2 = _BND_GRAM and os.environ.get("DPE_BND_GRAM_S2", "0") == "1"
_PW_FUSED_P = _GRAM and os.environ.get("DPE_PW_FUSED_P", "1") != "0"


def _ax_ok(conv, cin) -> bool:
    return (tuple(conv.kernel_size) == (1, 1) and tuple(conv.stride) == (1, 1) and tuple(conv.padding) == (0, 0)
            and cin % 32 == 0 and cin <= 2048)


def can_materialise_input(block) -> bool:
    return _AX_FWD and block.fused and _ax_ok(block.c1.conv, block.c1.conv.in_channels)


def _out_hw(hw, conv):
    k, s, p, d = conv.kernel_size[0], conv.stride[0], conv.padding[0], conv.dilation[0]
    return (hw + 2 * p - d * (k - 1) - 1) // s + 1


class _BN3Link:

    __slots__ = ("h3", "coef", "mask", "part", "dz_ptr", "dz_shape", "pending", "gram", "psrc", "P")

    def __init__(self):
        self.h3 = self.coef = self.mask = self.part = None
        self.psrc = self.P = None
        self.dz_ptr, self.dz_shape = 0, None
        self.gram = False
        self.pending = None


def _conv_conf(conv):
    return list(conv.stride), list(conv.padding), list(conv.dilation)


class BottleneckFn(Function):
    @staticmethod
    def forward(ctx, x, block, link_in, link_out, defer_out, gram_next, *params):
        C = ext()
        convs = [block.c1, block.c2, block.c3] + ([block.down] if block.down is not None else [])
        ws = [shadow(cb.conv.weight) for cb in convs]
        pend = link_in.pending if link_in is not None else None
        if pend is not None:
            ph3, pc3, pidn, pcd, pout, pbits = pend
            assert pout is x, "deferred block output consumed by a different tensor"
            link_in.pending = None
            h1_st = C.conv1x1_bnin_fwd(ph3, pidn, pc3, pcd, ws[0], x, pbits, True, _AX_TILE)
        else:
            h1_st = None

        def convbn(i, inp, relu, residual=None):
            cb = convs[i]
            s, p, d = _conv_conf(cb.conv)
            if i == 0 and h1_st is not None:
                h, st = h1_st
            else:
                h, st = C.conv_fwd(inp, ws[i], s, p, d, True, None)
            bn = cb.bn
            y, coef = C.bn_fwd_train(h, bn.weight.detach(), bn.bias.detach(), bn.running_mean, bn.running_var,
                                     bn.momentum, bn.eps, relu, residual, st)
            return h, y, coef

        def conv_coef(i, inp, in_coef=None):
            cb = convs[i]
            s, p, d = _conv_conf(cb.conv)
            if i == 0 and h1_st is not None:
                h, st = h1_st
            else:
                h, st = C.conv_fwd(inp, ws[i], s, p, d, True, None, in_coef)
            bn = cb.bn
            M = h.numel() // h.shape[-1]
            return h, C.bn_coef(st, M, bn.weight.detach(), bn.bias.detach(), bn.running_mean, bn.running_var, bn.momentum,
                                bn.eps)

        c1conv, c2conv = convs[0].conv, convs[1].conv
        if h1_st is None and block.down is not None:
            hd, cd = conv_coef(3, x)
        else:
            hd, cd = None, None
        h1_shape = [x.shape[0], _out_hw(x.shape[1], c1conv), _out_hw(x.shape[2], c1conv), c1conv.out_channels]
        if _ROW_BNIN and C.row_bn_on_load(h1_shape, list(ws[1].shape), *_conv_conf(c2conv)):
            h1, c1 = conv_coef(0, x)
            a1 = None
            h2, st2 = C.conv_fwd(h1, ws[1], *_conv_conf(c2conv), True, None, c1)
        else:
            h1, a1, c1 = convbn(0, x, True)
            h2, st2 = C.conv_fwd(a1, ws[1], *_conv_conf(c2conv), True, None)
        if h1_st is not None and block.down is not None:
            hd, cd = conv_coef(3, x)
        bn2 = convs[1].bn
        if _PW_BNIN and C.pw_bn_on_load(list(h2.shape), convs[2].conv.out_channels):
            c2 = C.bn_coef(st2, h2.numel() // h2.shape[-1], bn2.weight.detach(), bn2.bias.detach(),
                           bn2.running_mean, bn2.running_var, bn2.momentum, bn2.eps)
            a2 = None
        else:
            a2, c2 = C.bn_fwd_train(h2, bn2.weight.detach(), bn2.bias.detach(), bn2.running_mean,
                                    bn2.running_var, bn2.momentum, bn2.eps, True, None, st2)
        want_bits = True
        gram = None
        bnd = None
        out_shape = [*h2.shape[:3], convs[2].conv.out_channels]
        if (gram_next and link_out is not None and not defer_out and h1_st is None
                and (gram_next > 0 or C.pw_dgrad_strided_residual_ok(out_shape, -gram_next))
                and C.gram_ok(list(h2.shape), convs[2].conv.out_channels, abs(gram_next))):
            src, src_coef = (h2, c2) if a2 is None else (a2, None)
            G, sv = C.bn_gram(src, src_coef, c2)
            bn3 = convs[2].bn
            M3 = h2.numel() // h2.shape[-1]
            c3, u3 = C.bn_gram_coef(G, sv, ws[2], M3, bn3.weight.detach(), bn3.bias.detach(), bn3.running_mean,
                                    bn3.running_var, bn3.momentum, bn3.eps)
            if block.down is not None:
                out, bits = C.conv1x1_apply(src, ws[2], src_coef, c3, hd, cd)
            else:
                out, bits = C.conv1x1_apply(src, ws[2], src_coef, c3, x, None)
            h3 = None
            gram = (u3, sv, M3)
            dconv = block.down.conv if block.down is not None else None
            if (_BND_GRAM and dconv is not None and tuple(dconv.kernel_size) == (1, 1) and tuple(dconv.padding) == (0, 0)
                    and C.bnd_gram_ok(list(x.shape), dconv.out_channels, list(dconv.stride))
                    and (tuple(dconv.stride) == (1, 1) or (_BND_GRAM_S2 and tuple(convs[0].conv.stride) == (1, 1) and
                         C.pw_dgrad_strided_residual_ok(list(x.shape), convs[0].conv.out_channels)))):
                s2 = tuple(dconv.stride) == (2, 2)
                Gx, sx = C.bn_gram(x, None, C.bn_gram_pilot(x, s2), s2)
                bnd = (C.bn_gram_u(Gx, ws[3]), sx)
        else:
            h3, c3 = conv_coef(2, h2, c2) if a2 is None else conv_coef(2, a2)
        if gram is not None:
            pass
        elif defer_out and link_out is not None:
            out = torch.empty_like(h3)
            bits = torch.empty(*h3.shape[:-1], h3.shape[-1] // 8, dtype=torch.uint8, device=h3.device)
            link_out.pending = (h3, c3, hd, cd, out, bits) if block.down is not None else (h3, c3, x, None, out, bits)
        elif block.down is not None:
            out, bits = C.bn_apply(h3, c3, hd, cd, True, want_bits)
        else:
            out, bits = C.bn_apply(h3, c3, x, None, True, want_bits)
        ctx.save_for_backward(x, h1, a1, h2, a2, h3, out, None if bnd is not None else hd, c1, c2, c3, cd)
        strided_ok = block.down is not None and _DOWN_CHAIN and tuple(block.down.conv.stride) == (2, 2) and \
            tuple(block.down.conv.kernel_size) == (1, 1) and tuple(convs[0].conv.stride) == (1, 1) and \
            C.pw_dgrad_strided_residual_ok(list(x.shape), convs[0].conv.out_channels)
        ctx.link_in = (link_in if (link_in is not None and (block.down is None or strided_ok)
                                   and (link_in.h3 is not None or link_in.gram) and link_in.mask is not None) else None)
        if link_in is not None and link_in.gram and ctx.link_in is None:
            raise RuntimeError("BN3 Gram path: the next block cannot chain the BN3 backward "
                               f"(input {tuple(x.shape)}, downsample={block.down is not None})")
        ctx.link_out = link_out
        ctx.bits = bits
        ctx.gram = gram
        ctx.bnd = bnd
        if link_out is not None:
            link_out.h3, link_out.coef, link_out.mask = h3, c3, bits
            link_out.gram = gram is not None
            if gram is not None and _PW_FUSED_P:
                link_out.psrc = (h2, c2) if a2 is None else (a2, None)
            if gram is not None and block.down is not None and bnd is None:
                link_out.h3, link_out.coef = hd, cd
        ctx.block = block
        ctx.convs = convs
        ctx.ws = ws
        for cb in convs:
            note_use(cb.conv.weight)
            note_use(cb.bn.weight)
            note_use(cb.bn.bias)
        return out

    @staticmethod
    def backward(ctx, dout):
        C = ext()
        x, h1, a1, h2, a2, h3, out, hd, c1, c2, c3, cd = ctx.saved_tensors
        convs, ws = ctx.convs, ctx.ws
        has_down = len(convs) == 4
        dout = dout.contiguous()
        grads = {}
        res_mask = None
        dhd = None
        dh3_coef = None

        def bn_sinks(i):
            bn = convs[i].bn
            gb, gd = grad_sink(bn.weight)
            bb, bd = grad_sink(bn.bias)
            return bn, gb, gd, bb, bd

        def bn_done(bn, gb, gd, bb, bd):
            grad_done(bn.weight, gd)
            grad_done(bn.bias, bd)
            grads[id(bn.weight)] = None if gd else gb
            grads[id(bn.bias)] = None if bd else bb

        def bn_bwd(i, dy, y, h, coef, want_dz, y_bits=None):
            bn, gb, gd, bb, bd = bn_sinks(i)
            dh, dz = C.bn_bwd(dy, y, h, bn.weight.detach(), coef, gb, bb, want_dz, y_bits)
            bn_done(bn, gb, gd, bb, bd)
            return dh, dz

        def wgrad(i, dy, inp, in_coef=None):
            w = convs[i].conv.weight
            s, p, d = _conv_conf(convs[i].conv)
            buf, direct = grad_sink(w)
            if direct:
                fs = finalize_stream(dy.device)
                run_on_aux(dy.device, lambda: C.conv_wgrad(dy, inp, buf, s, p, d, 1.0, in_coef, fs), dy, inp, in_coef)
            else:
                C.conv_wgrad(dy, inp, buf, s, p, d, 1.0, in_coef)
            grad_done(w, direct)
            grads[id(w)] = None if direct else buf

        def dgrad(i, dy, shape, residual=None):
            s, p, d = _conv_conf(convs[i].conv)
            return C.conv_dgrad(dy, ws[i], shape, s, p, d, residual)

        def dgrad_bnb(i, dy, j, y, h, coef):
            if not _EPI_BNB:
                da = dgrad(i, dy, list(h.shape))
                return bn_bwd(j, da, y, h, coef, False)[0]
            s, p, d = _conv_conf(convs[i].conv)
            da, part = C.conv_dgrad_bn(dy, ws[i], list(h.shape), s, p, d, None, h, coef)
            bn, gb, gd, bb, bd = bn_sinks(j)
            dh = C.bn_bwd_partials(da, h, bn.weight.detach(), coef, part, gb, bb)
            bn_done(bn, gb, gd, bb, bd)
            return dh

        lk = ctx.link_out
        chained = (lk is not None and lk.part is not None and lk.dz_ptr == dout.data_ptr()
                   and lk.dz_shape == tuple(dout.shape))
        gram = ctx.gram
        ctx.gram = None
        if gram is not None:
            if not chained:
                raise RuntimeError("BN3 Gram path: the block output's gradient did not come from the chained epilogue")
            u3, sv, M3 = gram
            dz3 = dout
            src, src_coef = (h2, c2) if a2 is None else (a2, None)
            w3 = convs[2].conv.weight
            s3, p3, d3 = _conv_conf(convs[2].conv)
            P, lk.P, lk.psrc = lk.P, None, None
            if P is None:
                P = torch.empty(w3.shape, dtype=torch.float32, device=w3.device)
                C.conv_wgrad(dz3, src, P, s3, p3, d3, 1.0, src_coef, deterministic=True, overwrite=True)
            bn, gb, gd, bb, bd = bn_sinks(2)
            wbuf, wdirect = grad_sink(w3)
            bcat, ebias = C.bn_gram_bwd(lk.part, P, ws[2], u3, sv, c3, bn.weight.detach(), M3, gb, bb, wbuf)
            bn_done(bn, gb, gd, bb, bd)
            grad_done(w3, wdirect)
            grads[id(w3)] = None if wdirect else wbuf
            dhd = dxd = None
            bnd, ctx.bnd = ctx.bnd, None
            if bnd is not None:
                ud, sx = bnd
                wd = convs[3].conv.weight
                sd, pd, dd = _conv_conf(convs[3].conv)
                Pd = torch.empty(wd.shape, dtype=torch.float32, device=wd.device)
                C.conv_wgrad(dz3, x, Pd, sd, pd, dd, 1.0, None, deterministic=True, overwrite=True)
                bn, gb, gd, bb, bd = bn_sinks(3)
                dbuf, ddirect = grad_sink(wd)
                bcat_d, ebias_d = C.bn_gram_bwd(lk.part, Pd, ws[3], ud, sx, cd, bn.weight.detach(),
                                                dz3.numel() // dz3.shape[-1], gb, bb, dbuf)
                bn_done(bn, gb, gd, bb, bd)
                grad_done(wd, ddirect)
                grads[id(wd)] = None if ddirect else dbuf
                dxd = (C.conv1x1_dgrad_cat_plain(dz3, x, bcat_d, ebias_d, sd[0] == 2) if ctx.needs_input_grad[0]
                       else None)
            elif has_down and lk.h3 is not None:
                bn, gb, gd, bb, bd = bn_sinks(3)
                dhd = C.bn_bwd_partials(dz3, hd, bn.weight.detach(), cd, lk.part, gb, bb, relu_mask=False)
                bn_done(bn, gb, gd, bb, bd)
            lk.part = None
            lk.h3 = lk.coef = lk.mask = None
            ctx.bits = None
            da2, part2 = C.conv1x1_dgrad_cat(dz3, src, src_coef, bcat, ebias, h2, c2)
            bn, gb, gd, bb, bd = bn_sinks(1)
            dh2 = C.bn_bwd_partials(da2, h2, bn.weight.detach(), c2, part2, gb, bb)
            bn_done(bn, gb, gd, bb, bd)
            return BottleneckFn._backward_tail(ctx, C, dz3, None, dh2, grads, bn_sinks, bn_done, bn_bwd, wgrad, dgrad,
                                               dgrad_bnb, dhd, bnd is not None, dxd)
        if chained:
            dz3 = dout
            bn, gb, gd, bb, bd = bn_sinks(2)
            if has_down and _BN_DUAL:
                bnd, gbd, gdd, bbd, bdd = bn_sinks(3)
                dh3, dhd = C.bn_bwd_dual(dz3, h3, bn.weight.detach(), c3, lk.part, gb, bb, hd, bnd.weight.detach(), cd,
                                         gbd, bbd)
                bn_done(bnd, gbd, gdd, bbd, bdd)
            elif _AX_BWD and _EPI_BNB and h3.shape[-1] <= _AX_BWD_MAXC and _ax_ok(convs[2].conv, h3.shape[-1]):
                dh3_coef = C.bn_bwd_coef(lk.part, h3.numel() // h3.shape[-1], bn.weight.detach(), c3, gb, bb)
            else:
                dh3 = C.bn_bwd_partials(dz3, h3, bn.weight.detach(), c3, lk.part, gb, bb, relu_mask=False)
            bn_done(bn, gb, gd, bb, bd)
            lk.part = None
        elif ctx.bits is not None and not has_down:
            dh3, _ = bn_bwd(2, dout, out, h3, c3, False, ctx.bits)
            dz3, res_mask = dout, ctx.bits
        else:
            dh3, dz3 = bn_bwd(2, dout, out, h3, c3, True, ctx.bits)
        ctx.bits = None
        if lk is not None:
            lk.h3 = lk.coef = lk.mask = None
        if dh3_coef is not None:
            dh3 = torch.empty_like(h3)
            da2, part2 = C.conv1x1_bnin_dgrad(dz3, h3, dh3_coef, ws[2], dh3, h2, c2)
            bn, gb, gd, bb, bd = bn_sinks(1)
            dh2 = C.bn_bwd_partials(da2, h2, bn.weight.detach(), c2, part2, gb, bb)
            bn_done(bn, gb, gd, bb, bd)
            if a2 is None:
                wgrad(2, dh3, h2, c2)
            else:
                wgrad(2, dh3, a2)
        else:
            if a2 is None:
                wgrad(2, dh3, h2, c2)
            else:
                wgrad(2, dh3, a2)
            dh2 = dgrad_bnb(2, dh3, 1, a2, h2, c2)
        return BottleneckFn._backward_tail(ctx, C, dz3, res_mask, dh2, grads, bn_sinks, bn_done, bn_bwd, wgrad, dgrad,
                                           dgrad_bnb, dhd)

    @staticmethod
    def _dgrad_sum(C, li, dh1, w, xshape, s, p, d, residual, res_mask, res_s2):
        src = li.psrc
        if src is not None and C.pw_dgrad_fused_p_ok(xshape, w.shape[0], src[0].shape[-1]):
            dx, part, li.P = C.conv_dgrad_bn(dh1, w, xshape, s, p, d, residual, None, None, None, res_mask, res_s2,
                                             li.mask, p_src=src[0], p_coef=src[1])
            return dx, part
        return C.conv_dgrad_bn(dh1, w, xshape, s, p, d, residual, None, None, None, res_mask, res_s2, li.mask)

    @staticmethod
    def _backward_tail(ctx, C, dz3, res_mask, dh2, grads, bn_sinks, bn_done, bn_bwd, wgrad, dgrad, dgrad_bnb, dhd=None,
                       down_done=False, dxd=None):
        x, h1, a1, h2, a2, h3, out, hd, c1, c2, c3, cd = ctx.saved_tensors
        convs, ws = ctx.convs, ctx.ws
        has_down = len(convs) == 4
        if a1 is None:
            wgrad(1, dh2, h1, c1)
        else:
            wgrad(1, dh2, a1)
        dh1 = dgrad_bnb(1, dh2, 0, a1, h1, c1)
        wgrad(0, dh1, x)
        dx = None
        if down_done:
            s2 = convs[3].conv.stride[0] == 2
            li = ctx.link_in
            assert li is None or s2, "a stride-1 downsample block is never chained from the previous block"
            if dxd is None:
                pass
            elif not s2:
                dx = dgrad(0, dh1, list(x.shape), dxd)
            else:
                s, p, d = _conv_conf(convs[0].conv)
                if li is None:
                    dx = C.conv_dgrad_bn(dh1, ws[0], list(x.shape), s, p, d, dxd, None, None, None, None, True)[0]
                elif li.gram and li.h3 is None:
                    dx, part = BottleneckFn._dgrad_sum(C, li, dh1, ws[0], list(x.shape), s, p, d, dxd, None, True)
                else:
                    dx, part = C.conv_dgrad_bn(dh1, ws[0], list(x.shape), s, p, d, dxd, li.h3, li.coef, li.mask, None,
                                               True)
                if li is not None:
                    li.part, li.dz_ptr, li.dz_shape = part, dx.data_ptr(), tuple(dx.shape)
        elif ctx.needs_input_grad[0]:
            if has_down and ctx.link_in is not None:
                if dhd is None:
                    dhd, _ = bn_bwd(3, dz3, None, hd, cd, False)
                wgrad(3, dhd, x)
                li = ctx.link_in
                n, hh, ww, cin = x.shape
                dxd = C.conv_dgrad(dhd, ws[3], [n, hh // 2, ww // 2, cin], [1, 1], [0, 0], [1, 1])
                s, p, d = _conv_conf(convs[0].conv)
                if li.gram and li.h3 is None:
                    dx, part = BottleneckFn._dgrad_sum(C, li, dh1, ws[0], list(x.shape), s, p, d, dxd, None, True)
                else:
                    dx, part = C.conv_dgrad_bn(dh1, ws[0], list(x.shape), s, p, d, dxd, li.h3, li.coef, li.mask, None,
                                               True)
                li.part, li.dz_ptr, li.dz_shape = part, dx.data_ptr(), tuple(dx.shape)
            elif has_down:
                if dhd is None:
                    dhd, _ = bn_bwd(3, dz3, None, hd, cd, False)
                wgrad(3, dhd, x)
                dx = dgrad(0, dh1, list(x.shape))
                s, p, d = _conv_conf(convs[3].conv)
                C.conv_dgrad_acc(dhd, ws[3], dx, s, p, d)
            elif ctx.link_in is not None:
                li = ctx.link_in
                s, p, d = _conv_conf(convs[0].conv)
                if li.gram and li.h3 is None:
                    dx, part = BottleneckFn._dgrad_sum(C, li, dh1, ws[0], list(x.shape), s, p, d, dz3, res_mask, False)
                else:
                    dx, part = C.conv_dgrad_bn(dh1, ws[0], list(x.shape), s, p, d, dz3, li.h3, li.coef, li.mask, res_mask)
                li.part, li.dz_ptr, li.dz_shape = part, dx.data_ptr(), tuple(dx.shape)
            else:
                s, p, d = _conv_conf(convs[0].conv)
                dx = C.conv_dgrad(dh1, ws[0], list(x.shape), s, p, d, dz3, res_mask)
        elif has_down:
            if dhd is None:
                dhd, _ = bn_bwd(3, dz3, None, hd, cd, False)
            wgrad(3, dhd, x)
        pgrads = [grads.get(id(p)) for p in ctx.block._fused_params]
        return (dx, None, None, None, None, None, *pgrads)


def gram_successor_width(nxt) -> int:
    if not _GRAM or nxt is None or not nxt.fused:
        return 0
    c1 = nxt.c1.conv
    if tuple(c1.kernel_size) != (1, 1) or tuple(c1.stride) != (1, 1):
        return 0
    if nxt.down is not None:
        d = nxt.down.conv
        if not (_DOWN_CHAIN and tuple(d.stride) == (2, 2) and tuple(d.kernel_size) == (1, 1)):
            return 0
        return -c1.out_channels
    return c1.out_channels


def bottleneck_forward(block, x, link_in=None, chain=False, count_batches=True, defer_out=False, gram_next=0):
    params = block._fused_params
    if count_batches:
        nbt = [cb.bn.num_batches_tracked
               for cb in [block.c1, block.c2, block.c3] + ([block.down] if block.down is not None else [])]
        torch._foreach_add_(nbt, 1)
    link_out = _BN3Link() if (chain and _BN3_CHAIN) else None
    out = BottleneckFn.apply(x, block, link_in if _BN3_CHAIN else None, link_out, bool(defer_out and link_out is not None),
                             int(gram_next) if link_out is not None else 0, *params)
    return (out, link_out) if chain else out
```

Baseline: 17430 samples/s.

## Fuse stride-1 downsample conv into conv3 apply via concatenated-K streaming kernel

Adds a PW_CAT epilogue to the streaming pointwise kernel. It computes relu(BN3(a2 W3^T) + BN_d(x Wd^T)) in a single pass over the concatenated K, using two accumulators, and writes the ReLU bits. The downsample BN coefficients come from a Gram of x rather than a stored pre-BN downsample output, so the separate downsample conv and its output tensor are skipped on the forward path. The risks are extra register pressure from the second accumulator and the preloaded coefficients, and a fallback that recomputes hd with a separate conv when the Gram backward does not apply.

```diff
diff --git a/csrc/bindings/bn.cpp b/csrc/bindings/bn.cpp
--- a/csrc/bindings/bn.cpp
+++ b/csrc/bindings/bn.cpp
@@ -145,6 +145,43 @@
   pa.out_bits = (uint8_t*)bits.data_ptr();
   pa.M = M; pa.N = N; pa.K = K; pa.rg = rg; pa.sched = dpe_gemm::sched_buffer(cur_stream());
   CHECK_RC(dpe_pw_launch(&pa, dpe::PW_APPLY, cur_stream()), "pw_stream apply");
+  return {y, bits};
+}
+
+bool down_cat_ok(const std::vector<int64_t>& xshape, int64_t cmid, int64_t cout, int64_t stride) {
+  if (xshape.size() != 4 || stride != 1 || !pw_stream_on()) return false;
+  const int64_t M = xshape[0] * xshape[1] * xshape[2], C = xshape[3];
+  return (C == 64 || C == 128) && cmid == C && dpe_pw_cat_fwd_rowgroups(M, cout, C) > 0;
+}
+
+std::vector<Tensor> conv1x1_apply_cat(const Tensor& x, const Tensor& w, const c10::optional<Tensor>& in_coef,
+                                      const Tensor& out_coef, const Tensor& x2, const Tensor& w2, const Tensor& coef2) {
+  CHECK_GPU(x); CHECK_BF16(x); CHECK_CONTIG(x); CHECK_BF16(w); CHECK_CONTIG(w); CHECK_F32(out_coef); CHECK_CONTIG(out_coef);
+  CHECK_GPU(x2); CHECK_BF16(x2); CHECK_CONTIG(x2); CHECK_BF16(w2); CHECK_CONTIG(w2); CHECK_F32(coef2); CHECK_CONTIG(coef2);
+  const int64_t K1 = x.size(-1), M = x.numel() / K1, N = w.size(0), K2 = x2.size(-1);
+  TORCH_CHECK(x.dim() == 4 && K1 == K2 && x2.numel() == M * K2 && w.numel() == N * K1 && w2.numel() == N * K2 &&
+                  out_coef.numel() == 4 * N && coef2.numel() == 4 * N, "conv1x1_apply_cat: shapes");
+  if (has(in_coef)) {
+    CHECK_F32((*in_coef)); CHECK_CONTIG((*in_coef));
+    TORCH_CHECK(in_coef->numel() == 4 * K1, "conv1x1_apply_cat: in_coef must be the BN's [4][K] coefficients");
+  }
+  TORCH_CHECK(down_cat_ok(x2.sizes().vec(), K1, N, 1), "conv1x1_apply_cat: outside the envelope (down_cat_ok)");
+  const int rg = dpe_pw_cat_fwd_rowgroups(M, N, K2);
+  auto ysz = x.sizes().vec();
+  ysz.back() = N;
+  Tensor y = at::empty(ysz, x.options());
+  auto bsz = ysz;
+  bsz.back() = N / 8;
+  Tensor bits = at::empty(bsz, x.options().dtype(at::kByte));
+  dpe::PwArgs pa{};
+  pa.x = bp(x); pa.w = bp(w); pa.y = bpm(y);
+  pa.x2 = bp(x2); pa.w2 = bp(w2); pa.cat_k2 = (int)K2;
+  pa.in_coef = fpo(in_coef);
+  pa.out_coef = fp(out_coef);
+  pa.res_coef = fp(coef2);
+  pa.out_bits = (uint8_t*)bits.data_ptr();
+  pa.M = M; pa.N = N; pa.K = K1 + K2; pa.rg = rg; pa.sched = dpe_gemm::sched_buffer(cur_stream());
+  CHECK_RC(dpe_pw_launch(&pa, dpe::PW_CAT, cur_stream()), "pw_stream concatenated-K apply");
   return {y, bits};
 }
 
@@ -566,6 +603,11 @@
   m.def("conv1x1_apply", &conv1x1_apply, py::arg("x"), py::arg("w"), py::arg("in_coef"), py::arg("out_coef"),
         py::arg("residual"), py::arg("res_coef") = py::none(),
         "y = relu(BN(x' W^T) + residual [BN_d]) and its ReLU bits (pre-BN tensor never stored)");
+  m.def("conv1x1_apply_cat", &conv1x1_apply_cat, py::arg("x"), py::arg("w"), py::arg("in_coef"), py::arg("out_coef"),
+        py::arg("x2"), py::arg("w2"), py::arg("coef2"),
+        "y = relu(BN3(x' W^T) + BN_d(x2 W2^T)) over the concatenated K and its ReLU bits (no pre-BN tensors)");
+  m.def("down_cat_ok", &down_cat_ok, py::arg("xshape"), py::arg("cmid"), py::arg("cout"), py::arg("stride"),
+        "conv1x1_apply_cat's envelope: 1x1 stride-1 downsample conv, Cin == cmid in {64, 128}, cout == 4 Cin");
   m.def("bn_gram_bwd", &bn_gram_bwd, py::arg("part"), py::arg("P"), py::arg("w"), py::arg("u"), py::arg("s"),
         py::arg("coef"), py::arg("gamma"), py::arg("M"), py::arg("dgamma"), py::arg("dbeta"), py::arg("dw"),
         "BN3 backward from (sum dz partials, P = dz^T a2): dgamma/dbeta/dw +=, returns (B_cat bf16, bias)");
diff --git a/csrc/kernels/pwconv.h b/csrc/kernels/pwconv.h
--- a/csrc/kernels/pwconv.h
+++ b/csrc/kernels/pwconv.h
@@ -9,6 +9,7 @@
   PW_DGRAD = 1,
   PW_APPLY = 2,
   PW_DSUM = 3,
+  PW_CAT = 4,
 };
 
 struct PwArgs {
@@ -33,6 +34,9 @@
   const float* p_coef;
   float* p_slab;
   int p_k2;
+  const uint16_t* x2;
+  const uint16_t* w2;
+  int cat_k2;
 };
 
 struct PwCatArgs {
@@ -55,5 +59,7 @@
 extern "C" int dpe_pw_rowgroups(int64_t M, int64_t N, int64_t K, int epi);
 extern "C" int dpe_pw_launch(const dpe::PwArgs* args, int epi, hipStream_t stream);
 
+extern "C" int dpe_pw_cat_fwd_rowgroups(int64_t M, int64_t N, int64_t k2);
+
 extern "C" int dpe_pw_p_rowgroups(int64_t M, int64_t N, int64_t K, int64_t k2);
 extern "C" int dpe_pw_p_reduce(const float* slab, int rg, int64_t n, float* P, hipStream_t stream);
diff --git a/csrc/kernels/pwconv.hip b/csrc/kernels/pwconv.hip
--- a/csrc/kernels/pwconv.hip
+++ b/csrc/kernels/pwconv.hip
@@ -54,10 +54,14 @@
   static_assert(P >= 1 && P * 4096 == TILE, "pieces");
   constexpr int ROWB = WN * 2 + 16, CPRW = WN / 8, RPP = 64 / CPRW, NPS = 32 / RPP;
   constexpr int STG = 32 * ROWB;
-  constexpr int S = (EPI == PW_APPLY ? 4 : 2) * NPS;
+  constexpr int S = (EPI == PW_APPLY || EPI == PW_CAT ? 4 : 2) * NPS;
   constexpr int VM = (NS - 1) * S + (NS - 2) * P;
   static_assert(VM < 64, "vmcnt range");
-  constexpr bool PF = K2 > 0;
+  constexpr bool CAT = EPI == PW_CAT;
+  static_assert(!CAT || (WN == 32 && 2 * K2 == K && K2 % 64 == 0), "concatenated K: envelope");
+  constexpr int KS = CAT ? K2 : K;
+  constexpr int KC1 = KS / 32;
+  constexpr bool PF = K2 > 0 && !CAT;
   static_assert(!PF || (EPI == PW_DSUM && WN == 32 && (K2 == 64 || K2 == 128) && K2 <= K), "fused P: envelope");
   constexpr int A2OFF = NS * TILE + 4 * STG + 2 * K * 4 + 16, A2RB = 2 * (PF ? K2 : 8);
   __shared__ __attribute__((aligned(16))) char smem[A2OFF + (PF ? BM * A2RB : 0)];
@@ -84,7 +88,10 @@
 #pragma unroll
     for (int kc = 0; kc < KC; ++kc) {
       const int n = n0w + 16 * ni + li, k0 = 32 * kc + 8 * g;
-      if constexpr (!DG) {
+      if constexpr (CAT) {
+        const uint16_t* const ws = kc < KC1 ? a.w : a.w2;
+        wf[ni][kc] = __builtin_bit_cast(bf16x8, *(const u32x4*)(ws + (int64_t)n * KS + (k0 - (kc < KC1 ? 0 : KS))));
+      } else if constexpr (!DG) {
         wf[ni][kc] = __builtin_bit_cast(bf16x8, *(const u32x4*)(a.w + (int64_t)n * K + k0));
       } else {
         s16x8 v;
@@ -105,17 +112,18 @@
     }
   }
 
-  const __amdgpu_buffer_rsrc_t xr = rsrc(a.x, (uint32_t)((int64_t)M * K * 2));
+  const bool seg2 = CAT && wid >= 2;
+  const __amdgpu_buffer_rsrc_t xr = rsrc(seg2 ? a.x2 : a.x, (uint32_t)((int64_t)M * KS * 2));
   uint32_t voff[P];
 #pragma unroll
   for (int i = 0; i < P; ++i) {
     const int q = wid * P + i, kc = q >> 2, row = (q & 3) * 16 + (lane >> 2);
     const int lc = (lane & 3) ^ ((0x78 >> (((row >> 2) & 3) << 1)) & 3);
-    voff[i] = (uint32_t)(row * K * 2 + kc * 64 + lc * 16);
+    voff[i] = (uint32_t)(row * KS * 2 + (kc % KC1) * 64 + lc * 16);
   }
   auto issue = [&](int t, int slot) {
     char* dst = smem + slot * TILE;
-    const int64_t base = t >= 0 ? (int64_t)t * BM * K * 2 : 0;
+    const int64_t base = t >= 0 ? (int64_t)t * BM * KS * 2 : 0;
     const int valid_rows = t >= 0 ? M - t * BM : 0;
 #pragma unroll
     for (int i = 0; i < P; ++i) {
@@ -162,12 +170,24 @@
   const __amdgpu_buffer_rsrc_t rmrs = rsrc(a.res_mask, a.res_mask ? mbytes : 0u);
   const __amdgpu_buffer_rsrc_t xsrs = rsrc(a.st_x, bnx ? ybytes : 0u);
   const __amdgpu_buffer_rsrc_t smrs = rsrc(a.st_mask, (bnb && a.st_mask) ? mbytes : 0u);
-  const __amdgpu_buffer_rsrc_t obrs = rsrc(a.out_bits, (EPI == PW_APPLY && a.out_bits) ? mbytes : 0u);
+  const __amdgpu_buffer_rsrc_t obrs = rsrc(a.out_bits, ((EPI == PW_APPLY || CAT) && a.out_bits) ? mbytes : 0u);
   const __amdgpu_buffer_rsrc_t psrs = rsrc(a.p_src, PF ? (uint32_t)((int64_t)M * K2 * 2) : 0u);
 
   if (!DG && a.in_coef) {
-    for (int i = tid; i < 2 * K; i += 256) bnin[i] = a.in_coef[i];
+    for (int i = tid; i < 2 * KS; i += 256) bnin[i] = a.in_coef[i];
     __syncthreads();
+  }
+  float c1s[CAT ? NI : 1][4], c2s[CAT ? NI : 1][4], cbs[CAT ? NI : 1][4];
+  if constexpr (CAT) {
+#pragma unroll
+    for (int ni = 0; ni < NI; ++ni)
+#pragma unroll
+      for (int e = 0; e < 4; ++e) {
+        const int n = n0w + 16 * ni + 4 * g + e;
+        c1s[ni][e] = a.out_coef[n];
+        c2s[ni][e] = a.res_coef[n];
+        cbs[ni][e] = a.out_coef[N + n] + a.res_coef[N + n];
+      }
   }
   if constexpr (PF) {
     if (a.p_coef)
@@ -177,10 +197,11 @@
 
   auto tile_body = [&](const int m0, const int cur_slot, const int nxt_tile, const int nxt_slot) {
     constexpr bool HOIST = (EPI != PW_FWD) && (WN == 32);
-    constexpr int HN = HOIST ? NPS : 1;
+    constexpr bool HLD = HOIST && !CAT;
+    constexpr int HN = HLD ? NPS : 1;
     u32x4 hrv[2][HN], hxv[2][HN];
     uint32_t hrmb[2][HN], hsmb[2][HN];
-    if constexpr (HOIST) {
+    if constexpr (HLD) {
 #pragma unroll
       for (int hf = 0; hf < 2; ++hf)
 #pragma unroll
@@ -210,12 +231,12 @@
     if (!DG && a.in_coef) {
       char* timg = smem + cur_slot * TILE;
 #pragma unroll
-      for (int q = 0; q < TILE / 16 / 256; ++q) {
+      for (int q = 0; q < BM * KS * 2 / 16 / 256; ++q) {
         const int c = q * 256 + tid, kc = c / (BM * 4), rem = c % (BM * 4), row = rem >> 2, pc = rem & 3;
         const int lc = pc ^ ((0x78 >> (((row >> 2) & 3) << 1)) & 3);
         u32x4* pch = (u32x4*)(timg + kc * (BM * 64) + row * 64 + pc * 16);
         const f32x4* cs = (const f32x4*)(bnin + 32 * kc + 8 * lc);
-        const f32x4* chh = (const f32x4*)(bnin + K + 32 * kc + 8 * lc);
+        const f32x4* chh = (const f32x4*)(bnin + KS + 32 * kc + 8 * lc);
         const f32x4 s0 = cs[0], s1 = cs[1], h0 = chh[0], h1 = chh[1];
         const float sc8[8] = {s0[0], s0[1], s0[2], s0[3], s1[0], s1[1], s1[2], s1[3]};
         const float sh8[8] = {h0[0], h0[1], h0[2], h0[3], h1[0], h1[1], h1[2], h1[3]};
@@ -234,6 +255,13 @@
     for (int mi = 0; mi < MI; ++mi)
 #pragma unroll
       for (int ni = 0; ni < NI; ++ni) acc[mi][ni] = f32x4{0.f, 0.f, 0.f, 0.f};
+    f32x4 acc2[CAT ? MI : 1][CAT ? NI : 1];
+    if constexpr (CAT) {
+#pragma unroll
+      for (int mi = 0; mi < MI; ++mi)
+#pragma unroll
+        for (int ni = 0; ni < NI; ++ni) acc2[mi][ni] = f32x4{0.f, 0.f, 0.f, 0.f};
+    }
 #pragma unroll
     for (int kc = 0; kc < KC; ++kc) {
       bf16x8 xf[MI];
@@ -242,8 +270,15 @@
 #pragma unroll
       for (int mi = 0; mi < MI; ++mi)
 #pragma unroll
-        for (int ni = 0; ni < NI; ++ni)
+        for (int ni = 0; ni < NI; ++ni) {
+          if constexpr (CAT) {
+            if (kc >= KC1) {
+              acc2[mi][ni] = __builtin_amdgcn_mfma_f32_16x16x32_bf16(wf[ni][kc], xf[mi], acc2[mi][ni], 0, 0, 0);
+              continue;
+            }
+          }
           acc[mi][ni] = __builtin_amdgcn_mfma_f32_16x16x32_bf16(wf[ni][kc], xf[mi], acc[mi][ni], 0, 0, 0);
+        }
     }
     if constexpr (PF) {
       wait_vm<P>();
@@ -272,7 +307,7 @@
     for (int hf = 0; hf < 2; ++hf) {
       u32x4 rv[NPS], xv[NPS];
       uint32_t rmb[NPS], smb[NPS];
-      if constexpr (HOIST) {
+      if constexpr (HLD) {
 #pragma unroll
         for (int ps = 0; ps < HN; ++ps) {
           rv[ps] = hrv[hf][ps];
@@ -299,13 +334,18 @@
         const int mi = 2 * hf + mh;
 #pragma unroll
         for (int ni = 0; ni < NI; ++ni) {
+          if constexpr (CAT) {
+#pragma unroll
+            for (int e = 0; e < 4; ++e)
+              acc[mi][ni][e] = fmaxf(fmaf(acc[mi][ni][e], c1s[ni][e], fmaf(acc2[mi][ni][e], c2s[ni][e], cbs[ni][e])), 0.f);
+          }
           u32x2 pk;
           pk[0] = pack_bf2(acc[mi][ni][0], acc[mi][ni][1]);
           pk[1] = pack_bf2(acc[mi][ni][2], acc[mi][ni][3]);
           *(u32x2*)(stg + (16 * mh + li) * ROWB + (16 * ni + 4 * g) * 2) = pk;
         }
       }
-      if (HOIST && hf == 0) wait_vm<P>();
+      if (HLD && hf == 0) wait_vm<P>();
 #pragma unroll
       for (int ps = 0; ps < NPS; ++ps) {
         const int row = ps * RPP + lane / CPRW;
@@ -328,6 +368,8 @@
             __builtin_amdgcn_raw_buffer_store_b8(relu_mask_byte(v), obrs, valid ? (uint32_t)(((int64_t)m * N + nch) >> 3) : OOB, 0, 0);
           else if (valid && a.out_bits)
             a.out_bits[((int64_t)m * N + nch) >> 3] = relu_mask_byte(v);
+        } else if constexpr (CAT) {
+          __builtin_amdgcn_raw_buffer_store_b8(relu_mask_byte(v), obrs, valid ? (uint32_t)(((int64_t)m * N + nch) >> 3) : OOB, 0, 0);
         } else if constexpr (EPI == PW_FWD) {
           const float vm = valid ? 1.f : 0.f;
 #pragma unroll
@@ -396,7 +438,7 @@
     if constexpr (PF) asm volatile("s_waitcnt lgkmcnt(0)" ::: "memory");
   };
   auto flush_stats = [&](int col) {
-    if (EPI != PW_APPLY && a.stats) {
+    if (EPI != PW_APPLY && !CAT && a.stats) {
 #pragma unroll
       for (int e = 0; e < 8; ++e) {
 #pragma unroll
@@ -716,7 +758,7 @@
 #define DPE_PW128_FWD_WN 64
 #endif
 static int pw_wn(int K, int epi) {
-  if (epi == PW_APPLY) return 32;
+  if (epi == PW_APPLY || epi == PW_CAT) return 32;
   if (epi == PW_DSUM) epi = PW_DGRAD;
   if (K == 64) return epi == PW_DGRAD ? DPE_PW64_DGRAD_WN : DPE_PW64_FWD_WN;
   if (K == 128) return epi == PW_FWD ? DPE_PW128_FWD_WN : 32;
@@ -762,8 +804,15 @@
   return 0;
 }
 
+static bool pw_cat_shape(int64_t K, int64_t k2) { return (K == 128 && k2 == 64) || (K == 256 && k2 == 128); }
+template <bool DYN>
+static int pw_cap_cat(int64_t K) {
+  return K == 128 ? pw_slots<128, 32, 3, PW_CAT, DYN, 64>() : pw_slots<256, 32, 2, PW_CAT, DYN, 128>();
+}
+
 template <bool DYN>
 static int pw_cap(int64_t K, int epi, int64_t k2 = 0) {
+  if (epi == PW_CAT) return pw_cap_cat<DYN>(K);
   if (k2 > 0) return pw_cap_p<DYN>(K, k2);
   return epi == PW_FWD ? pw_capacity<PW_FWD, DYN>((int)K)
                        : epi == PW_APPLY ? pw_capacity<PW_APPLY, DYN>((int)K)
@@ -772,9 +821,13 @@
 
 struct PwPlan { int rg, srg; };
 static PwPlan pw_plan(int64_t M, int64_t N, int64_t K, int epi, int64_t k2 = 0) {
-  if (k2 > 0 && (epi != PW_DSUM || !pw_p_shape(K, k2))) return {0, 0};
+  if (epi == PW_CAT) {
+    if (!pw_cat_shape(K, k2)) return {0, 0};
+  } else if (k2 > 0 && (epi != PW_DSUM || !pw_p_shape(K, k2))) {
+    return {0, 0};
+  }
   if (K != 64 && K != 128 && K != 256) return {0, 0};
-  if (epi != PW_FWD && epi != PW_DGRAD && epi != PW_APPLY && epi != PW_DSUM) return {0, 0};
+  if (epi != PW_FWD && epi != PW_DGRAD && epi != PW_APPLY && epi != PW_DSUM && epi != PW_CAT) return {0, 0};
   const int bnb = 4 * pw_wn((int)K, epi);
   if (N % bnb || N < 2 * K) return {0, 0};
   if (M * K * 2 >= (1ll << 31) - 4096 || M * N >= (1ll << 31) - 256) return {0, 0};
@@ -782,7 +835,7 @@
   const int64_t nbN = N / bnb;
   const int reserve = dpe_cu_reserve();
   if (reserve > 0 && pw_dynamic()) {
-    if (k2 == 128) return {0, 0};
+    if (k2 == 128 && epi != PW_CAT) return {0, 0};
     const int64_t srg = std::max<int64_t>(1, (pw_cap<true>(K, epi, k2) - reserve) / nbN);
     static const int64_t fac = [] { const char* e = getenv("DPE_PW_DYN_FACTOR"); return (int64_t)(e ? std::max(2, atoi(e)) : 8); }();
     const int64_t rg = std::min<int64_t>(fac * srg, tiles / 7);
@@ -794,6 +847,10 @@
 }
 
 extern "C" int dpe_pw_rowgroups(int64_t M, int64_t N, int64_t K, int epi) { return pw_plan(M, N, K, epi).rg; }
+
+extern "C" int dpe_pw_cat_fwd_rowgroups(int64_t M, int64_t N, int64_t k2) {
+  return (k2 > 0 && N == 4 * k2) ? pw_plan(M, N, 2 * k2, PW_CAT, k2).rg : 0;
+}
 
 extern "C" int dpe_pw_p_rowgroups(int64_t M, int64_t N, int64_t K, int64_t k2) {
   return k2 > 0 ? pw_plan(M, N, K, PW_DSUM, k2).rg : 0;
@@ -835,14 +892,19 @@
 extern "C" int dpe_pw_launch(const PwArgs* args, int epi, hipStream_t st) {
   const PwArgs& a = *args;
   if (a.p_k2 < 0 || (a.p_k2 > 0 && (epi != PW_DSUM || !a.p_src || !a.p_slab))) return -1;
-  if (a.rg <= 0 || a.rg != pw_plan(a.M, a.N, a.K, epi, a.p_k2).rg) return -1;
+  if ((epi == PW_CAT) != (a.cat_k2 > 0) || (epi == PW_CAT && a.p_k2 > 0)) return -1;
+  const int64_t k2 = epi == PW_CAT ? a.cat_k2 : a.p_k2;
+  if (a.rg <= 0 || a.rg != pw_plan(a.M, a.N, a.K, epi, k2).rg) return -1;
+  if (epi == PW_CAT && (!a.x2 || !a.w2 || !a.out_coef || !a.res_coef || !a.out_bits || a.residual || a.st_x || a.stats ||
+                        a.res_h > 0))
+    return -1;
   if (epi == PW_FWD && (a.residual || a.st_x)) return -1;
   if (a.st_x && !a.st_coef) return -1;
   if (epi == PW_DSUM && (a.st_x || !a.st_mask || !a.stats)) return -1;
   if (epi == PW_APPLY && (!a.out_coef || a.st_x || a.stats || a.res_h > 0 || (a.res_coef && !a.residual))) return -1;
   if (a.res_h > 0 && ((epi != PW_DGRAD && epi != PW_DSUM) || a.res_mask || a.res_h % 2 || a.res_w % 2 || a.M % ((int64_t)a.res_h * a.res_w)))
     return -1;
-  const int srg = a.sched ? pw_plan(a.M, a.N, a.K, epi, a.p_k2).srg : a.rg;
+  const int srg = a.sched ? pw_plan(a.M, a.N, a.K, epi, k2).srg : a.rg;
   const bool dyn = srg < a.rg;
   const int wn = pw_wn((int)a.K, epi);
   const dim3 grid((unsigned)(srg * (a.N / (4 * wn)))), block(256);
@@ -858,6 +920,16 @@
     else hipLaunchKernelGGL((pw::pw_stream_kernel<K_, 32, NS_, PW_DSUM, false, K2_>), grid, block, 0, st, a);     \
     return 0;                                                                                              \
   }
+  if (epi == PW_CAT) {
+    if (a.K == 128) {
+      if (dyn) hipLaunchKernelGGL((pw::pw_stream_kernel<128, 32, 3, PW_CAT, true, 64>), grid, block, 0, st, a);
+      else hipLaunchKernelGGL((pw::pw_stream_kernel<128, 32, 3, PW_CAT, false, 64>), grid, block, 0, st, a);
+    } else {
+      if (dyn) hipLaunchKernelGGL((pw::pw_stream_kernel<256, 32, 2, PW_CAT, true, 128>), grid, block, 0, st, a);
+      else hipLaunchKernelGGL((pw::pw_stream_kernel<256, 32, 2, PW_CAT, false, 128>), grid, block, 0, st, a);
+    }
+    return 0;
+  }
   if (a.p_k2 > 0) {
     PW_GO_P(64, 4, 64) PW_GO_P(128, 3, 64)
     if (a.K == 128 && a.p_k2 == 128 && !dyn) {
diff --git a/distributed_pytorch_example_amd/models/_resnet_fused.py b/distributed_pytorch_example_amd/models/_resnet_fused.py
--- a/distributed_pytorch_example_amd/models/_resnet_fused.py
+++ b/distributed_pytorch_example_amd/models/_resnet_fused.py
@@ -22,6 +22,7 @@
 _BND_GRAM = _GRAM and os.environ.get("DPE_BND_GRAM", "1") != "0"
 _BND_GRAM_S2 = _BND_GRAM and os.environ.get("DPE_BND_GRAM_S2", "0") == "1"
 _PW_FUSED_P = _GRAM and os.environ.get("DPE_PW_FUSED_P", "1") != "0"
+_DOWN_CAT =_BND_GRAM and os.environ.get("DPE_DOWN_CAT", "1") != "0"
 
 
 def _ax_ok(conv, cin) -> bool:
@@ -94,11 +95,25 @@
                                 bn.eps)
 
         c1conv, c2conv = convs[0].conv, convs[1].conv
-        if h1_st is None and block.down is not None:
+        h1_shape = [x.shape[0], _out_hw(x.shape[1], c1conv), _out_hw(x.shape[2], c1conv), c1conv.out_channels]
+        h2_shape = [x.shape[0], _out_hw(h1_shape[1], c2conv), _out_hw(h1_shape[2], c2conv), c2conv.out_channels]
+        out_shape = [*h2_shape[:3], convs[2].conv.out_channels]
+        dconv = block.down.conv if block.down is not None else None
+        use_gram = bool(gram_next and link_out is not None and not defer_out and h1_st is None
+                        and (gram_next > 0 or C.pw_dgrad_strided_residual_ok(out_shape, -gram_next))
+                        and C.gram_ok(h2_shape, convs[2].conv.out_channels, abs(gram_next)))
+        bnd_gram = bool(use_gram and _BND_GRAM and dconv is not None and tuple(dconv.kernel_size) == (1, 1)
+                        and tuple(dconv.padding) == (0, 0)
+                        and C.bnd_gram_ok(list(x.shape), dconv.out_channels, list(dconv.stride))
+                        and (tuple(dconv.stride) == (1, 1) or (_BND_GRAM_S2 and tuple(c1conv.stride) == (1, 1) and
+                             C.pw_dgrad_strided_residual_ok(list(x.shape), c1conv.out_channels))))
+        down_cat = bool(use_gram and _DOWN_CAT and dconv is not None and tuple(dconv.kernel_size) == (1, 1)
+                        and tuple(dconv.padding) == (0, 0) and tuple(dconv.stride) == (1, 1)
+                        and C.down_cat_ok(list(x.shape), h2_shape[3], dconv.out_channels, 1))
+        if h1_st is None and block.down is not None and not down_cat:
             hd, cd = conv_coef(3, x)
         else:
             hd, cd = None, None
-        h1_shape = [x.shape[0], _out_hw(x.shape[1], c1conv), _out_hw(x.shape[2], c1conv), c1conv.out_channels]
         if _ROW_BNIN and C.row_bn_on_load(h1_shape, list(ws[1].shape), *_conv_conf(c2conv)):
             h1, c1 = conv_coef(0, x)
             a1 = None
@@ -119,27 +134,31 @@
         want_bits = True
         gram = None
         bnd = None
-        out_shape = [*h2.shape[:3], convs[2].conv.out_channels]
-        if (gram_next and link_out is not None and not defer_out and h1_st is None
-                and (gram_next > 0 or C.pw_dgrad_strided_residual_ok(out_shape, -gram_next))
-                and C.gram_ok(list(h2.shape), convs[2].conv.out_channels, abs(gram_next))):
+        assert list(h2.shape) == h2_shape
+        if use_gram:
             src, src_coef = (h2, c2) if a2 is None else (a2, None)
             G, sv = C.bn_gram(src, src_coef, c2)
             bn3 = convs[2].bn
             M3 = h2.numel() // h2.shape[-1]
             c3, u3 = C.bn_gram_coef(G, sv, ws[2], M3, bn3.weight.detach(), bn3.bias.detach(), bn3.running_mean,
                                     bn3.running_var, bn3.momentum, bn3.eps)
-            if block.down is not None:
+            if down_cat:
+                bnd_ = convs[3].bn
+                Gx, sx = C.bn_gram(x, None, C.bn_gram_pilot(x, False), False)
+                cd, ud = C.bn_gram_coef(Gx, sx, ws[3], M3, bnd_.weight.detach(), bnd_.bias.detach(), bnd_.running_mean,
+                                        bnd_.running_var, bnd_.momentum, bnd_.eps)
+                out, bits = C.conv1x1_apply_cat(src, ws[2], src_coef, c3, x, ws[3], cd)
+                if bnd_gram:
+                    bnd = (ud, sx)
+                else:
+                    hd = C.conv_fwd(x, ws[3], *_conv_conf(dconv), False, None)[0]
+            elif block.down is not None:
                 out, bits = C.conv1x1_apply(src, ws[2], src_coef, c3, hd, cd)
             else:
                 out, bits = C.conv1x1_apply(src, ws[2], src_coef, c3, x, None)
             h3 = None
             gram = (u3, sv, M3)
-            dconv = block.down.conv if block.down is not None else None
-            if (_BND_GRAM and dconv is not None and tuple(dconv.kernel_size) == (1, 1) and tuple(dconv.padding) == (0, 0)
-                    and C.bnd_gram_ok(list(x.shape), dconv.out_channels, list(dconv.stride))
-                    and (tuple(dconv.stride) == (1, 1) or (_BND_GRAM_S2 and tuple(convs[0].conv.stride) == (1, 1) and
-                         C.pw_dgrad_strided_residual_ok(list(x.shape), convs[0].conv.out_channels)))):
+            if bnd_gram and not down_cat:
                 s2 = tuple(dconv.stride) == (2, 2)
                 Gx, sx = C.bn_gram(x, None, C.bn_gram_pilot(x, s2), s2)
                 bnd = (C.bn_gram_u(Gx, ws[3]), sx)
```

Result: faster. 17640 samples/s, median of 6 (+1.2%).
